# xcompact3d/x3d2

Hardware: AMD Instinct MI355X
Metric: DoF*steps/s (whole node), TGV 512^3 per GPU, full fractional step (higher is better)
Workload: dtype f64; 1 GPU; TGV 512x512x512 all-periodic, Re=1600, dt=1e-3, RK3 (3 substeps/step), compact6/classic schemes, rocFFT Poisson (configs[2]); per_gpu=512^3, driver=fused, parallelism=domain decomposition 1x1x1, decomposition=yslabs, decomposition_requested=auto, poisson_z_first=228

## Files before the change

### include/x3d2_hip.h

```cpp
#ifndef X3D2_HIP_H
#define X3D2_HIP_H

#include <stddef.h>

#ifdef X3D_SINGLE_PREC
typedef float x3d_real;
#else
typedef double x3d_real;
#endif

#ifdef __cplusplus
extern "C" {
#endif

enum { X3D_DIR_X = 1, X3D_DIR_Y = 2, X3D_DIR_Z = 3, X3D_DIR_C = 4 };
enum { X3D_BC_PERIODIC = 0, X3D_BC_NEUMANN = 1, X3D_BC_DIRICHLET = 2, X3D_BC_HALO = -1 };
enum { X3D_X_FACE = 1100, X3D_Y_FACE = 1010, X3D_Z_FACE = 110 };
#define X3D_N_HALO 4

typedef struct x3d_backend x3d_backend;
typedef struct x3d_tdsops x3d_tdsops;
typedef struct x3d_poisson x3d_poisson;

const char *x3d_last_error(void);
// ... 198 lines not shown
int x3d_poisson_postprocess_010(x3d_poisson *p);
int x3d_poisson_solve_010(x3d_poisson *p, x3d_real *f, x3d_real *temp);
int x3d_poisson_solve_010_rows(x3d_poisson *p, x3d_real *f);
int x3d_transpose_xy(x3d_backend *b_src, x3d_backend *b_dst, x3d_real *dst, const x3d_real *src, int nx, int ny, int nz);
int x3d_transpose_xyz_zxy(x3d_backend *b_src, x3d_backend *b_dst, x3d_real *dst, const x3d_real *src, int nx, int ny, int nz);
int x3d_transpose_zxy_xyz(x3d_backend *b_src, x3d_backend *b_dst, x3d_real *dst, const x3d_real *src, int nx, int ny, int nz);
int x3d_poisson_enforce_periodicity_z(x3d_poisson *p, x3d_real *f_out, const x3d_real *f_in);
int x3d_poisson_undo_periodicity_z(x3d_poisson *p, x3d_real *f_out, const x3d_real *f_in);
int x3d_poisson_postprocess_011(x3d_poisson *p);
int x3d_poisson_get_spectral(x3d_poisson *p, x3d_real *host_interleaved);
int x3d_poisson_set_spectral(x3d_poisson *p, const x3d_real *host_interleaved);

typedef struct x3d_sfft x3d_sfft;
int x3d_sfft_create(x3d_backend *b, x3d_sfft **out, const int nglob[3], int pz, int rz);
int x3d_sfft_destroy(x3d_sfft *p);
int x3d_sfft_sizes(const x3d_sfft *p, long out[4]);
int x3d_sfft_set_waves(x3d_sfft *p, const x3d_real *waves, const x3d_real *ax, const x3d_real *bx, const x3d_real *ay,
                       const x3d_real *by, const x3d_real *az, const x3d_real *bz);
int x3d_sfft_forward_local(x3d_sfft *p, const x3d_real *f_in, x3d_real *sendbuf);
int x3d_sfft_fft_z(x3d_sfft *p, x3d_real *recvbuf, int dir);
int x3d_sfft_postprocess_000(x3d_sfft *p, x3d_real *recvbuf);
int x3d_sfft_backward_local(x3d_sfft *p, const x3d_real *recvbuf, x3d_real *f_out);
int x3d_sfft_create_parts(x3d_backend *b, x3d_sfft **out, const int nglob[3], int pz, int rz, int parts);
int x3d_sfft_fft_z_part(x3d_sfft *p, x3d_real *recvbuf, int dir, int part);
int x3d_sfft_postprocess_000_part(x3d_sfft *p, x3d_real *recvbuf, int part);

typedef struct x3d_sfft010 x3d_sfft010;
int x3d_sfft010_create(x3d_backend *b, x3d_sfft010 **out, const int nglob_cell[3], int pz, int rz);
int x3d_sfft010_destroy(x3d_sfft010 *p);
int x3d_sfft010_sizes(const x3d_sfft010 *p, long out[6]);
int x3d_sfft010_create_parts(x3d_backend *b, x3d_sfft010 **out, const int nglob_cell[3], int pz, int rz, int parts);
int x3d_sfft010_fft_z_part(x3d_sfft010 *p, x3d_real *recvbuf, int dir, int part);
int x3d_sfft010_postprocess_010_part(x3d_sfft010 *p, x3d_real *recvbuf, int part);
int x3d_sfft010_set_waves(x3d_sfft010 *p, const x3d_real *waves, const x3d_real *ax, const x3d_real *bx, const x3d_real *ay,
                          const x3d_real *by, const x3d_real *az, const x3d_real *bz);
int x3d_sfft010_set_stretching(x3d_sfft010 *p, int sym, const x3d_real *a0, const x3d_real *a1);
int x3d_sfft010_periodicity_y(x3d_sfft010 *p, x3d_real *f_out, const x3d_real *f_in, int undo);
int x3d_sfft010_forward_local(x3d_sfft010 *p, const x3d_real *f_in, x3d_real *sendbuf);
int x3d_sfft010_fft_z(x3d_sfft010 *p, x3d_real *recvbuf, int dir);
int x3d_sfft010_postprocess_010(x3d_sfft010 *p, x3d_real *recvbuf);
int x3d_sfft010_backward_local(x3d_sfft010 *p, const x3d_real *sendbuf, x3d_real *f_out);

int x3d_poisson_zfirst_ok(x3d_poisson *p, int *ok);
int x3d_tds_pair_zfirst_ok(x3d_backend *b, const x3d_tdsops *ta, const x3d_tdsops *tb, int *ok);
int x3d_poisson_zfirst_middle(x3d_poisson *p);
int x3d_poisson_zfirst_forward(x3d_poisson *p, const x3d_real *f_in);
int x3d_poisson_zfirst_backward(x3d_poisson *p, x3d_real *f_out);
int x3d_poisson_solve_000_zfirst(x3d_poisson *p, x3d_real *f);
int x3d_tds_solve_xfft_ok(x3d_backend *b, const x3d_tdsops *t, int *ok);
int x3d_tds_solve_xfft(x3d_backend *b, x3d_real *du, const x3d_real *u, const x3d_tdsops *t);
int x3d_poisson_xfft_ok(x3d_poisson *p, int *ok);
int x3d_poisson_zfirst_middle_xpacked(x3d_poisson *p);
int x3d_c2c512_x_rows(x3d_backend *b, x3d_real *c, long nrows, long pitch, int mode);
int x3d_poisson_set_stretching_zfirst(x3d_poisson *p, int sym, const x3d_real *a0, const x3d_real *a1);
int x3d_poisson_create_proxy(x3d_backend *b, x3d_poisson **out, x3d_real *spectrum, int ny, long px, int (*middle)(void *user),
                             void *user);
int x3d_poisson_solve_010_rows_zfirst(x3d_poisson *p, x3d_real *f);
int x3d_tds_pair_zfirst(x3d_backend *b, x3d_poisson *poisson, int mode, x3d_real *out1, x3d_real *out2, const x3d_real *in1,
                        const x3d_real *in2, const x3d_tdsops *ta, const x3d_tdsops *tb, int *done);

typedef struct x3d_sfftz x3d_sfftz;
int x3d_sfftz_create(x3d_backend *b, x3d_sfftz **out, const int nglob_cell[3], int py, int ry, int parts);
int x3d_sfftz_destroy(x3d_sfftz *p);
int x3d_sfftz_sizes(const x3d_sfftz *p, long out[16]);
int x3d_sfftz_spectrum(const x3d_sfftz *p, x3d_real **c, int *ny, long *px);
int x3d_sfftz_set_waves(x3d_sfftz *p, const x3d_real *rw, const x3d_real *ax, const x3d_real *bx, const x3d_real *ay,
                        const x3d_real *by, const x3d_real *az, const x3d_real *bz);
int x3d_sfftz_tds_pair(x3d_sfftz *p, int mode, x3d_real *out1, x3d_real *out2, const x3d_real *in1, const x3d_real *in2,
                       const x3d_tdsops *ta, const x3d_tdsops *tb, int *done);
int x3d_sfftz_z(x3d_sfftz *p, x3d_real *f, int inverse);
int x3d_sfftz_z_field(x3d_sfftz *p, x3d_real *f, int inverse);
int x3d_sfftz_x_forward(x3d_sfftz *p, x3d_real *sendbuf, int part);
int x3d_sfftz_y_stage(x3d_sfftz *p, x3d_real *recvbuf, int part, int what);
int x3d_sfftz_x_backward(x3d_sfftz *p, const x3d_real *buf, int part);
int x3d_sfftz_tds_pair_rows(x3d_sfftz *p, int mode, x3d_real *out1, x3d_real *out2, const x3d_real *in1, const x3d_real *in2,
                            const x3d_tdsops *ta, const x3d_tdsops *tb, int y0, int nyr, int *done);
int x3d_sfftz_z_rows(x3d_sfftz *p, x3d_real *f, int inverse, int y0, int nyr);
int x3d_sfftz_x_forward_rows(x3d_sfftz *p, x3d_real *sendbuf, int part, int y0, int nyr);
int x3d_sfftz_x_backward_rows(x3d_sfftz *p, const x3d_real *buf, int part, int y0, int nyr);

typedef struct x3d_pfft x3d_pfft;
int x3d_pfft_create(x3d_backend *b, x3d_pfft **out, const int nglob_cell[3], int py, int pz, int ry, int rz);
int x3d_pfft_destroy(x3d_pfft *p);
int x3d_pfft_sizes(const x3d_pfft *p, long out[8]);
int x3d_pfft_set_waves(x3d_pfft *p, const x3d_real *waves_re, const x3d_real *ax, const x3d_real *bx,
                       const x3d_real *ay, const x3d_real *by, const x3d_real *az, const x3d_real *bz);
int x3d_pfft_fwd_x(x3d_pfft *p, const x3d_real *f_in);
int x3d_pfft_bwd_x(x3d_pfft *p, x3d_real *f_out);
int x3d_pfft_fft_y(x3d_pfft *p, int inverse);
int x3d_pfft_fft_z(x3d_pfft *p, int inverse);
int x3d_pfft_pack_xy(x3d_pfft *p, x3d_real *sendbuf);
int x3d_pfft_unpack_xy(x3d_pfft *p, const x3d_real *recvbuf);
int x3d_pfft_pack_yx(x3d_pfft *p, x3d_real *sendbuf);
int x3d_pfft_unpack_yx(x3d_pfft *p, const x3d_real *recvbuf);
int x3d_pfft_pack_yz(x3d_pfft *p, x3d_real *sendbuf);
int x3d_pfft_unpack_yz(x3d_pfft *p, const x3d_real *recvbuf);
int x3d_pfft_pack_zy(x3d_pfft *p, x3d_real *sendbuf);
int x3d_pfft_unpack_zy(x3d_pfft *p, const x3d_real *recvbuf);
int x3d_pfft_transpose_local(x3d_pfft *p, int which);
int x3d_pfft_own_chunk(x3d_pfft *p, const x3d_real *sendbuf, int rank);
int x3d_pfft_postprocess_000(x3d_pfft *p);
int x3d_pfft_create_parts(x3d_backend *b, x3d_pfft **out, const int nglob_cell[3], int py, int pz, int ry, int rz,
                          int parts);
int x3d_pfft_part_layout(const x3d_pfft *p, long out[6]);
int x3d_pfft_fwd_a_part(x3d_pfft *p, const x3d_real *f_in, x3d_real *send_xy, int m);
int x3d_pfft_fwd_b_part(x3d_pfft *p, const x3d_real *recv_xy, x3d_real *send_yz, int m);
// ... 128 lines not shown
```

### x3d2_amd/_lib.py

```python
import ctypes
import os
import subprocess

from .common import X3dError

HERE = os.path.dirname(os.path.abspath(__file__))
SINGLE = os.environ.get("X3D_SINGLE_PREC") == "1"
LIB_PATH = os.path.join(HERE, "libx3d2_hip_sp.so" if SINGLE else "libx3d2_hip.so")
CSRC = os.path.join(HERE, "csrc")

REAL = ctypes.c_float if SINGLE else ctypes.c_double
NP_REAL = "float32" if SINGLE else "float64"
c_double_p = ctypes.POINTER(REAL)
c_int_p = ctypes.POINTER(ctypes.c_int)
VP = ctypes.c_void_p
I, D, SZT = ctypes.c_int, REAL, ctypes.c_size_t


def torch_real():
    import torch
    return torch.float32 if SINGLE else torch.float64

PROTOTYPES = {
    "x3d_last_error": (ctypes.c_char_p, []),
# ... 108 lines not shown
    "x3d_get_field_data_pitched": (I, [VP, c_double_p, VP, I, I, c_int_p]),
    "x3d_poisson_create": (I, [VP, ctypes.POINTER(VP), c_int_p] + [c_double_p] * 7),
    "x3d_poisson_destroy": (I, [VP]),
    "x3d_poisson_fft_forward": (I, [VP, VP]),
    "x3d_poisson_postprocess_000": (I, [VP]),
    "x3d_poisson_fft_backward": (I, [VP, VP]),
    "x3d_poisson_solve_000": (I, [VP, VP]),
    "x3d_poisson_enforce_periodicity_y": (I, [VP, VP, VP]),
    "x3d_poisson_undo_periodicity_y": (I, [VP, VP, VP]),
    "x3d_poisson_set_stretching": (I, [VP, ctypes.c_int, c_double_p, c_double_p]),
    "x3d_sfftz_spectrum": (I, [VP, ctypes.POINTER(VP), c_int_p, ctypes.POINTER(ctypes.c_long)]),
    "x3d_poisson_create_proxy": (I, [VP, ctypes.POINTER(VP), VP, I, ctypes.c_long, VP, VP]),
    "x3d_poisson_set_stretching_zfirst": (I, [VP, ctypes.c_int, c_double_p, c_double_p]),
    "x3d_poisson_postprocess_010": (I, [VP]),
    "x3d_poisson_solve_010": (I, [VP, VP, VP]),
    "x3d_poisson_solve_010_rows": (I, [VP, VP]),
    "x3d_poisson_solve_010_rows_zfirst": (I, [VP, VP]),
    "x3d_poisson_get_spectral": (I, [VP, c_double_p]),
    "x3d_poisson_set_spectral": (I, [VP, c_double_p]),
    "x3d_sfft_create": (I, [VP, ctypes.POINTER(VP), c_int_p, I, I]),
    "x3d_sfft_create_parts": (I, [VP, ctypes.POINTER(VP), c_int_p, I, I, I]),
    "x3d_sfft_fft_z_part": (I, [VP, VP, I, I]),
    "x3d_sfft_postprocess_000_part": (I, [VP, VP, I]),
    "x3d_sfft_destroy": (I, [VP]),
    "x3d_sfft_sizes": (I, [VP, ctypes.POINTER(ctypes.c_long)]),
    "x3d_sfft_set_waves": (I, [VP] + [c_double_p] * 7),
    "x3d_sfft_forward_local": (I, [VP, VP, VP]),
    "x3d_sfft_fft_z": (I, [VP, VP, I]),
    "x3d_sfft_postprocess_000": (I, [VP, VP]),
    "x3d_sfft_backward_local": (I, [VP, VP, VP]),
    "x3d_sfft010_create": (I, [VP, ctypes.POINTER(VP), c_int_p, I, I]),
    "x3d_sfft010_create_parts": (I, [VP, ctypes.POINTER(VP), c_int_p, I, I, I]),
    "x3d_sfft010_fft_z_part": (I, [VP, VP, I, I]),
    "x3d_sfft010_postprocess_010_part": (I, [VP, VP, I]),
    "x3d_sfft010_destroy": (I, [VP]),
    "x3d_sfft010_sizes": (I, [VP, ctypes.POINTER(ctypes.c_long)]),
    "x3d_sfft010_set_waves": (I, [VP] + [c_double_p] * 7),
    "x3d_sfft010_set_stretching": (I, [VP, I, c_double_p, c_double_p]),
    "x3d_sfft010_periodicity_y": (I, [VP, VP, VP, I]),
    "x3d_sfft010_forward_local": (I, [VP, VP, VP]),
    "x3d_sfft010_fft_z": (I, [VP, VP, I]),
    "x3d_sfft010_postprocess_010": (I, [VP, VP]),
    "x3d_sfft010_backward_local": (I, [VP, VP, VP]),
    "x3d_poisson_zfirst_ok": (I, [VP, c_int_p]),
    "x3d_poisson_zfirst_middle": (I, [VP]),
    "x3d_poisson_zfirst_forward": (I, [VP, VP]),
    "x3d_poisson_zfirst_backward": (I, [VP, VP]),
    "x3d_poisson_solve_000_zfirst": (I, [VP, VP]),
    "x3d_tds_solve_xfft_ok": (I, [VP, VP, c_int_p]),
    "x3d_tds_solve_xfft": (I, [VP, VP, VP, VP]),
    "x3d_poisson_xfft_ok": (I, [VP, c_int_p]),
    "x3d_poisson_zfirst_middle_xpacked": (I, [VP]),
    "x3d_c2c512_x_rows": (I, [VP, VP, ctypes.c_long, ctypes.c_long, I]),
    "x3d_tds_pair_zfirst": (I, [VP, VP, I, VP, VP, VP, VP, VP, VP, c_int_p]),
    "x3d_sfftz_create": (I, [VP, ctypes.POINTER(VP), c_int_p, I, I, I]),
    "x3d_sfftz_destroy": (I, [VP]),
    "x3d_sfftz_sizes": (I, [VP, ctypes.POINTER(ctypes.c_long)]),
    "x3d_sfftz_set_waves": (I, [VP] + [c_double_p] * 7),
    "x3d_sfftz_tds_pair": (I, [VP, I, VP, VP, VP, VP, VP, VP, c_int_p]),
    "x3d_sfftz_z": (I, [VP, VP, I]),
    "x3d_sfftz_z_field": (I, [VP, VP, I]),
    "x3d_sfftz_x_forward": (I, [VP, VP, I]),
    "x3d_sfftz_y_stage": (I, [VP, VP, I, I]),
    "x3d_sfftz_x_backward": (I, [VP, VP, I]),
    "x3d_sfftz_tds_pair_rows": (I, [VP, I, VP, VP, VP, VP, VP, VP, I, I, c_int_p]),
    "x3d_sfftz_z_rows": (I, [VP, VP, I, I, I]),
    "x3d_sfftz_x_forward_rows": (I, [VP, VP, I, I, I]),
    "x3d_sfftz_x_backward_rows": (I, [VP, VP, I, I, I]),
    "x3d_pfft_create": (I, [VP, ctypes.POINTER(VP), c_int_p, I, I, I, I]),
    "x3d_pfft_destroy": (I, [VP]),
    "x3d_pfft_sizes": (I, [VP, ctypes.POINTER(ctypes.c_long)]),
    "x3d_pfft_set_waves": (I, [VP] + [c_double_p] * 7),
    "x3d_pfft_fwd_x": (I, [VP, VP]),
    "x3d_pfft_bwd_x": (I, [VP, VP]),
    "x3d_pfft_fft_y": (I, [VP, I]),
    "x3d_pfft_fft_z": (I, [VP, I]),
    "x3d_pfft_pack_xy": (I, [VP, VP]),
    "x3d_pfft_unpack_xy": (I, [VP, VP]),
    "x3d_pfft_pack_yx": (I, [VP, VP]),
    "x3d_pfft_unpack_yx": (I, [VP, VP]),
    "x3d_pfft_pack_yz": (I, [VP, VP]),
    "x3d_pfft_unpack_yz": (I, [VP, VP]),
    "x3d_pfft_pack_zy": (I, [VP, VP]),
    "x3d_pfft_unpack_zy": (I, [VP, VP]),
    "x3d_pfft_transpose_local": (I, [VP, I]),
    "x3d_pfft_own_chunk": (I, [VP, VP, I]),
    "x3d_pfft_postprocess_000": (I, [VP]),
    "x3d_pfft_create_parts": (I, [VP, ctypes.POINTER(VP), c_int_p, I, I, I, I, I]),
    "x3d_pfft_part_layout": (I, [VP, ctypes.POINTER(ctypes.c_long)]),
    "x3d_pfft_fwd_a_part": (I, [VP, VP, VP, I]),
    "x3d_pfft_fwd_b_part": (I, [VP, VP, VP, I]),
    "x3d_pfft_fwd_c_part": (I, [VP, VP, I]),
    "x3d_pfft_bwd_c_part": (I, [VP, VP, I]),
    "x3d_pfft_bwd_b_part": (I, [VP, VP, VP, I]),
    "x3d_pfft_bwd_a_part": (I, [VP, VP, VP, I]),
    "x3d_stats_update_uvw": (I, [VP, VP, VP, VP, ctypes.POINTER(VP), D]),
    "x3d_stats_update_scalar": (I, [VP, VP, VP, VP, D]),
    "x3d_stats_derive": (I, [VP, ctypes.POINTER(VP), ctypes.POINTER(VP)]),
    "x3d_stats_profile_sums": (I, [VP, VP, VP, VP, c_int_p, I, VP]),
    "x3d_stats_profile_accumulate": (I, [VP, VP, VP, ctypes.c_long, D, D]),
    "x3d_ibm_create": (I, [VP, c_double_p, c_int_p, ctypes.POINTER(VP)]),
    "x3d_ibm_destroy": (I, [VP]),
    "x3d_ibm_counts": (I, [VP, ctypes.POINTER(ctypes.c_long)]),
    "x3d_ibm_body": (I, [VP, VP, VP, VP, VP, c_int_p]),
    "x3d_ibm_set_weights": (I, [VP] + [ctypes.POINTER(ctypes.c_double)] * 3),
    "x3d_ibm_body_loads": (I, [VP, VP, VP, VP, VP, c_int_p, VP, I]),
# ... 96 lines not shown
```

### x3d2_amd/backend.py

```python
import ctypes

import numpy as np
import torch

from . import _lib
from .common import (CELL, DIR_C, DIR_X, DIR_Y, DIR_Z, N_HALO, NULL_LOC, VERT, X_FACE, Y_FACE, Z_FACE, X3dError,
                     get_rdr_from_dirs, move_data_loc)
from .field import Allocator
from .parallel import Comm
from .switches import Switches
from .tdsops import Tdsops

VP = ctypes.c_void_p


def _dp(a):
    if a.dtype != np.dtype(_lib.NP_REAL):
        a = np.ascontiguousarray(a, dtype=_lib.NP_REAL)
    return a.ctypes.data_as(_lib.c_double_p)


class HipBackend:
    n_halo = N_HALO

# ... 415 lines not shown
            else:
                for j in jobs:
                    self.tds_job_local(direction, j)
                if after_lead:
                    after_lead()
            if between:
                between()
            return
        if direction != DIR_X and all(self.tds_tile_ok(direction, j, True, yperm=yperm) for j in jobs):
            hs = [self.tds_halo_begin(direction, j, k) for k, j in enumerate(jobs)]
            hb = [self.tds_halo_main(direction, j, k, hs[k], yperm=yperm) for k, j in enumerate(jobs)]
            if after_lead:
                after_lead()
            if between:
                between()
            for k, j in enumerate(jobs):
                self.tds_halo_finish(direction, j, k, hb[k], yperm=yperm)
            return
        if yperm:
            raise X3dError("tds_jobs: interleaved rows need the halo form of the z pairs (tds_tile_ok)")
        for j in jobs:
            self.tds_job_local(direction, j)
        if after_lead:
            after_lead()
        if between:
            between()

    def halo_strip_rows(self, *ops):
        out = (ctypes.c_int * 2)()
        ws = we = 0
        for t in ops:
            _lib.check(self.lib.x3d_tdsops_halo_rows(t.handle, out))
            ws, we = max(ws, out[0]), max(we, out[1])
        return ws, we

    def transeq_dir(self, direction, du, dv, dw, u, v, w, nu, dirps, accumulate=False):
        if not self._decomposed(direction):
            _lib.check(self.lib.x3d_transeq_acc(self.h, direction, du.ptr, dv.ptr, dw.ptr, u.ptr, v.ptr, w.ptr,
                                                float(nu), dirps.der1st.handle, dirps.der1st_sym.handle,
                                                dirps.der2nd.handle, dirps.der2nd_sym.handle, int(accumulate)))
            return
        self._transeq_dist(direction, du, dv, dw, u, v, w, nu, dirps, accumulate=accumulate)

    def transeq_x_update(self, du, dv, dw, u, v, w, nu, dirps, grads, op_u, op_vw, scale):
        if self._decomposed(DIR_X):
            return False
        flag = ctypes.c_int(0)
        _lib.check(self.lib.x3d_transeq_x_update(self.h, du.ptr, dv.ptr, dw.ptr, u.ptr, v.ptr, w.ptr, float(nu),
                                                 dirps.der1st.handle, dirps.der1st_sym.handle, dirps.der2nd.handle,
                                                 dirps.der2nd_sym.handle, grads[0].ptr, grads[1].ptr, grads[2].ptr,
                                                 op_u.handle, op_vw.handle, float(scale), ctypes.byref(flag)))
        return bool(flag.value)

    def transeq_x_update_rot(self, du, dv, dw, u, v, w, nu, dirps, grads, op_u, op_vw, scale, omega, u_shift=None):
        if self._decomposed(DIR_X):
            return False
        flag = ctypes.c_int(0)
        _lib.check(self.lib.x3d_transeq_x_update_rot(self.h, du.ptr, dv.ptr, dw.ptr, u.ptr, v.ptr, w.ptr, float(nu),
                                                     dirps.der1st.handle, dirps.der1st_sym.handle, dirps.der2nd.handle,
                                                     dirps.der2nd_sym.handle, grads[0].ptr, grads[1].ptr, grads[2].ptr,
                                                     op_u.handle, op_vw.handle, float(scale), float(omega), u_shift,
                                                     ctypes.byref(flag)))
        return bool(flag.value)

    def transeq_x_rot(self, du, dv, dw, u, v, w, nu, dirps, omega, u_shift=None):
        if self._decomposed(DIR_X):
            return False
        flag = ctypes.c_int(0)
        _lib.check(self.lib.x3d_transeq_x_rot(self.h, du.ptr, dv.ptr, dw.ptr, u.ptr, v.ptr, w.ptr, float(nu),
                                              dirps.der1st.handle, dirps.der1st_sym.handle, dirps.der2nd.handle,
                                              dirps.der2nd_sym.handle, float(omega), u_shift, ctypes.byref(flag)))
        return bool(flag.value)

    def transeq_dir_defer(self, direction, pend, u, v, w, nu, dirps):
        if self._decomposed(direction):
            return False
        flag = ctypes.c_int(0)
        _lib.check(self.lib.x3d_transeq_defer(self.h, direction, pend[0].ptr, pend[1].ptr, pend[2].ptr, u.ptr, v.ptr,
                                              w.ptr, float(nu), dirps.der1st.handle, dirps.der1st_sym.handle,
                                              dirps.der2nd.handle, dirps.der2nd_sym.handle, ctypes.byref(flag)))
        return bool(flag.value)

    def transeq_stage_ok(self, direction, dirps):
        if self._decomposed(direction):
            return False
        return bool(self.lib.x3d_transeq_stage_ok(self.h, direction, dirps.der1st.handle, dirps.der1st_sym.handle,
                                                  dirps.der2nd.handle, dirps.der2nd_sym.handle))

    def transeq_lincomb(self, direction, kind, u_ptr, conv_ptr, nu, dirps, y, base, coeffs, xs, ipend, store):
        n = len(xs)
        c = (_lib.REAL * n)(*[float(v) for v in coeffs])
        p = (VP * n)(*[x.ptr for x in xs])
        _lib.check(self.lib.x3d_transeq_lincomb(self.h, direction, int(kind), u_ptr, conv_ptr, float(nu),
                                                dirps.der1st.handle, dirps.der1st_sym.handle, dirps.der2nd.handle,
                                                dirps.der2nd_sym.handle, y.ptr, base.ptr, n, c, p, int(ipend),
                                                int(bool(store))))
        self.rk_fused_passes = getattr(self, "rk_fused_passes", 0) + n + 1
        self.rk_fused_launches = getattr(self, "rk_fused_launches", 0) + 1

    def transeq_lincomb3(self, direction, rhs, vel, nu, dirps, specs):
        y = (VP * 3)(*[sp[0].ptr for sp in specs])
        base = (VP * 3)(*[sp[1].ptr for sp in specs])
        nterm = _lib.ints(*[len(sp[3]) for sp in specs])
        c = (_lib.REAL * 15)()
        x = (VP * 15)()
        ipend, store = [], []
# ... 65 lines not shown
            if mode == 0:
                self.tds_apply(out1, in2, t_b, direction, accumulate=True)
            else:
                self.tds_apply(out2, in1, t_b, direction)
            return
        _lib.check(self.lib.x3d_tds_solve_pair(self.h, direction, int(mode), out1.ptr,
                                               out2.ptr if out2 is not None else None, in1.ptr,
                                               in2.ptr if in2 is not None else None, t_a.handle, t_b.handle))

    def tds_pair_yperm(self, mode, out1, out2, in1, in2, t_a, t_b, ny):
        if self._decomposed(DIR_Z) or self.sw.no_yperm:
            return False
        flag = ctypes.c_int(0)
        _lib.check(self.lib.x3d_tds_solve_pair_yperm(self.h, int(mode), out1.ptr,
                                                     out2.ptr if out2 is not None else None, in1.ptr,
                                                     in2.ptr if in2 is not None else None, t_a.handle, t_b.handle,
                                                     int(ny), ctypes.byref(flag)))
        return bool(flag.value)

    def tds_pair_zfirst(self, mode, out1, out2, in1, in2, t_a, t_b):
        if self._decomposed(DIR_Z) or self.poisson_fft is None or not hasattr(self.poisson_fft, "zfirst_ok"):
            return False
        if hasattr(self.poisson_fft, "zfirst_pair"):
            return self.poisson_fft.zfirst_pair(mode, out1, out2, in1, in2, t_a, t_b)
        flag = ctypes.c_int(0)
        ptr = lambda f: f.ptr if f is not None else None
        _lib.check(self.lib.x3d_tds_pair_zfirst(self.h, self.poisson_fft.h, int(mode), ptr(out1), ptr(out2), ptr(in1),
                                                ptr(in2), t_a.handle, t_b.handle, ctypes.byref(flag)))
        return bool(flag.value)

    def zfirst_pairs_ok(self, t_a, t_b):
        flag = ctypes.c_int(0)
        _lib.check(self.lib.x3d_tds_pair_zfirst_ok(self.h, t_a.handle, t_b.handle, ctypes.byref(flag)))
        return bool(flag.value)

    def tds_apply_mean(self, du, u, tdsops, direction, mean_target):
        if u.data_loc == NULL_LOC:
            raise X3dError("You must set the data_loc before calling volume integral.")
        out = VP()
        ncell = float(np.prod(self.mesh.get_global_dims(CELL)))
        _lib.check(self.lib.x3d_tds_solve_mean(self.h, du.ptr, u.ptr, tdsops.handle, direction, self._dims(u.data_loc), ncell,
                                               float(mean_target), ctypes.byref(out)))
        return out

    def tds_apply_xfft_ok(self, tdsops):
        if self._decomposed(DIR_X):
            return False
        flag = ctypes.c_int(0)
        _lib.check(self.lib.x3d_tds_solve_xfft_ok(self.h, tdsops.handle, ctypes.byref(flag)))
        return bool(flag.value)

    def tds_apply_xfft(self, du, u, tdsops):
        _lib.check(self.lib.x3d_tds_solve_xfft(self.h, du.ptr, u.ptr, tdsops.handle))

    def tds_apply(self, du, u, tdsops, direction, accumulate=False, scale=1.0):
        if not self._decomposed(direction):
            _lib.check(self.lib.x3d_tds_solve_acc(self.h, du.ptr, u.ptr, tdsops.handle, direction,
                                                  int(accumulate), float(scale)))
            return
        self._tds_dist(du, u, tdsops, direction, accumulate=accumulate, scale=scale)

    def tds_solve(self, du, u, tdsops):
        if u.dir != du.dir:
            raise X3dError("DIR mismatch between fields in tds_solve.")
        if u.data_loc != NULL_LOC:
            du.set_data_loc(move_data_loc(u.data_loc, u.dir, tdsops.move))
        direction = u.dir
        if direction == DIR_C:
            raise X3dError("tds_solve needs a directional field")
        if tdsops.pentadiag:
            self.tds_penta_solve(du, u, tdsops, direction)
            return
        if not self._decomposed(direction):
            _lib.check(self.lib.x3d_tds_solve(self.h, du.ptr, u.ptr, tdsops.handle, direction))
            return
        self._tds_dist(du, u, tdsops, direction)

    def tds_penta_solve(self, du, u, tdsops, direction, u_s=None, u_e=None):
        if self._decomposed(direction):
            raise X3dError("compact10_penta is a rank-local solve: the direction must not be decomposed")
        _lib.check(self.lib.x3d_tds_penta_solve(self.h, du.ptr, u.ptr, tdsops.handle, direction,
                                                u_s.data_ptr() if u_s is not None else None,
                                                u_e.data_ptr() if u_e is not None else None))

    def _tds_dist(self, du, u, tdsops, direction, accumulate=False, scale=1.0):
        if not accumulate and direction != DIR_X:
            job = (2, du, None, u, None, tdsops, None)
            if self.tds_tile_ok(direction, job, True):
                h = self.tds_halo_begin(direction, job, 0)
                hb = self.tds_halo_main(direction, job, 0, h)
                self.tds_halo_finish(direction, job, 0, hb)
                return
        d = direction - 1
        prev, nxt = int(self.mesh.pprev[d]), int(self.mesh.pnext[d])
        ss, se, rs, re = self._buffers(direction, N_HALO, "u0")
        _lib.check(self.lib.x3d_pack_halos(self.h, ss.data_ptr(), se.data_ptr(), u.ptr, tdsops.n_tds,
                                           direction))
        self.comm.sendrecv([(ss, se, rs, re)], prev, nxt)
        bs, be, brs, bre = self._buffers(direction, 1, "b1")
        _lib.check(self.lib.x3d_tds_dist_fwd(self.h, du.ptr, bs.data_ptr(), be.data_ptr(), u.ptr,
                                             rs.data_ptr(), re.data_ptr(), tdsops.handle, direction))
        self.comm.sendrecv([(bs, be, brs, bre)], prev, nxt)
        _lib.check(self.lib.x3d_tds_dist_bwd_acc(self.h, du.ptr, bs.data_ptr(), brs.data_ptr(), bre.data_ptr(),
                                                 tdsops.handle, direction, int(bool(accumulate)), float(scale)))

    def reorder(self, u_, u, direction):
# ... 423 lines not shown
```

### x3d2_amd/csrc/common.h

```cpp
#pragma once
#include <hip/hip_runtime.h>

#include <cstdarg>
#include <cstdio>
#include <cstring>
#include <vector>

#include "../../include/x3d2_hip.h"

typedef x3d_real real_t;
#ifdef X3D_SINGLE_PREC
typedef float2 real2_t;
#define make_real2 make_float2
#else
typedef double2 real2_t;
#define make_real2 make_double2
#endif
#ifdef X3D_SINGLE_PREC
#define X3D_FFT_R2C HIPFFT_R2C
#define X3D_FFT_C2R HIPFFT_C2R
#define X3D_FFT_C2C HIPFFT_C2C
#define x3d_fftExecR2C hipfftExecR2C
#define x3d_fftExecC2R hipfftExecC2R
#define x3d_fftExecC2C hipfftExecC2C
// ... 32 lines not shown
            x3d_set_error(__VA_ARGS__);                                                        \
            return 2;                                                                          \
        }                                                                                      \
    } while (0)

__device__ __forceinline__ double fma_r(double a, double b, double c) { return __builtin_fma(a, b, c); }
__device__ __forceinline__ float fma_r(float a, float b, float c) { return __builtin_fmaf(a, b, c); }

__device__ __forceinline__ void wave_lds_fence()
{
    __builtin_amdgcn_fence(__ATOMIC_RELEASE, "wavefront");
    __builtin_amdgcn_wave_barrier();
    __builtin_amdgcn_fence(__ATOMIC_ACQUIRE, "wavefront");
}

typedef real_t x3d_d2v __attribute__((ext_vector_type(2)));
__device__ __forceinline__ real2_t ldg_stream(const real2_t *p)
{
    const x3d_d2v v = __builtin_nontemporal_load(reinterpret_cast<const x3d_d2v *>(p));
    return make_real2(v.x, v.y);
}
__device__ __forceinline__ void stg_stream(real2_t *p, real2_t v)
{
    const x3d_d2v w = {v.x, v.y};
    __builtin_nontemporal_store(w, reinterpret_cast<x3d_d2v *>(p));
}

static __device__ __attribute__((used)) float g_vmcnt_sink[32 * 1024];
template <int N>
__device__ __forceinline__ void vmcnt_pad_stores()
{
#pragma unroll
    for (int k = 0; k < N; k++) __builtin_nontemporal_store(0.0f, &g_vmcnt_sink[k * 1024 + (threadIdx.x & 1023)]);
}

__host__ __device__ static inline unsigned long long x3d_mix64(unsigned long long z)
{
    z += 0x9E3779B97F4A7C15ull;
    z = (z ^ (z >> 30)) * 0xBF58476D1CE4E5B9ull;
    z = (z ^ (z >> 27)) * 0x94D049BB133111EBull;
    return z ^ (z >> 31);
}

struct PencilGeom {
    int np;
    int dim0;
    long s0, s1, rs;
};

#define X3D_SW_UNSET (-0x7fffffffL - 1)
struct x3d_switches {
    long no_via_x, no_xscan, no_ygen, no_ytile, no_q5, no_direct, sfft010_split_xy;
    long no_circ, no_halo_circ, no_uniform, xscan_p1, no_ztile, no_tds_pair, no_npw2, no_tile3, xdir_generic, no_xcirc;
    long no_tds_lincomb, no_zfirst010, no_zfirst, no_xwide, no_xwide_upd, no_xfft_div;
    long no_spectral_pad, no_fft512, no_rwt, no_r2c512, no_y010, y010_no_db, no_onchip2, no_slab_fused_z;
    long lazy_dump, lazy_report, lazy_keep_zero_terms;
    long pad_x;
    long slab_z_split;
    long lazy_rules;
    long y010_form;
    long via_x;
    long ytile;
    long ygen;
    long x_fast;
    long x_tq3;
    long x_circ;
};
void x3d_switches_from_env(x3d_switches *sw);

struct x3d_backend {
    x3d_switches sw;
    int device;
    hipStream_t stream;
    int nx, ny, nz;
    int ring[4];
    int nxp, nyp, nzp;
    size_t nblock;
    real_t *send_s, *send_e;
    real_t *scratch[3];
    real_t *red_buf;
    real_t *red_host;
    int red_cap;
    long n_upd;
    long n_tq3;
    long n_halo;
    void *epi_dev;
    hipEvent_t ev0, ev1;
    void *ipc_maps;
    struct x3d_prof *prof;
    unsigned prof_mask;
    int pair_yperm;
    void *lds_optin;
    struct x3d_lazy *lazy;
    int comm_reserve;
    double *stats_part;
    long stats_cap;
    real_t *bc_params;
    double *bc_part;
    long n_sync;
    void *snap;
};
void x3d_snapshot_destroy_c(x3d_backend *b);
int x3d_snapshot_wait_for_copy_c(x3d_backend *b, const void *dev);
int x3d_reduce_abs_partials_c(x3d_backend *b, const real_t *f, const int dims[3], int *nparts);
#define X3D_BC_PARTS 1024
struct TileEpi {
    real_t *y;
// ... 175 lines not shown
```

### x3d2_amd/csrc/fft512_core.h

```cpp
#pragma once
#include "common.h"

#define FP 584

__device__ __forceinline__ real2_t cmul(real2_t a, real2_t b)
{
    return make_real2(a.x * b.x - a.y * b.y, a.x * b.y + a.y * b.x);
}
__device__ __forceinline__ real2_t cadd(real2_t a, real2_t b) { return make_real2(a.x + b.x, a.y + b.y); }
__device__ __forceinline__ real2_t csub(real2_t a, real2_t b) { return make_real2(a.x - b.x, a.y - b.y); }

template <int S>
__device__ __forceinline__ void fft8(real2_t (&a)[8])
{
    const real_t h = 0.70710678118654752440;
    real2_t b[8];
#pragma unroll
    for (int k = 0; k < 4; k++) {
        b[k] = cadd(a[k], a[k + 4]);
        b[k + 4] = csub(a[k], a[k + 4]);
    }
    {
        real2_t t = b[5];
        b[5] = make_real2(h * (t.x - S * t.y), h * (t.y + S * t.x));
// ... 66 lines not shown
{
    const real2_t b0 = cadd(a[0], a[2]), b1 = csub(a[0], a[2]), b2 = cadd(a[1], a[3]), d = csub(a[1], a[3]);
    const real2_t b3 = make_real2(-S * d.y, S * d.x);
    a[0] = cadd(b0, b2);
    a[2] = csub(b0, b2);
    a[1] = cadd(b1, b3);
    a[3] = csub(b1, b3);
}

template <int S>
__device__ __forceinline__ void fft256_wave(real2_t (&a)[4], real2_t *__restrict__ pen, const real2_t *__restrict__ tw,
                                            int l)
{
    wave_lds_fence();
    fft4<S>(a);
#pragma unroll
    for (int f = 1; f < 4; f++) a[f] = cmul(a[f], twiddle<S>(tw, 2 * l * f));
#pragma unroll
    for (int f = 0; f < 4; f++) pen[f * 68 + l] = a[f];
    wave_lds_fence();
    {
        const int f1 = l >> 4, l0 = l & 15;
#pragma unroll
        for (int j = 0; j < 4; j++) a[j] = pen[f1 * 68 + l0 + 16 * j];
        fft4<S>(a);
#pragma unroll
        for (int f = 1; f < 4; f++) a[f] = cmul(a[f], twiddle<S>(tw, 8 * l0 * f));
        wave_lds_fence();
#pragma unroll
        for (int f = 0; f < 4; f++) pen[(f1 * 4 + f) * 17 + l0] = a[f];
    }
    wave_lds_fence();
    {
        const int r = l >> 2, m0 = l & 3;
#pragma unroll
        for (int m = 0; m < 4; m++) a[m] = pen[r * 17 + m0 + 4 * m];
        fft4<S>(a);
#pragma unroll
        for (int f = 1; f < 4; f++) a[f] = cmul(a[f], twiddle<S>(tw, 32 * m0 * f));
        wave_lds_fence();
#pragma unroll
        for (int f = 0; f < 4; f++) pen[(r * 4 + f) * 4 + m0 + (r >> 2) * 4] = a[f];
    }
    wave_lds_fence();
    {
        const int f1 = l & 3, f2 = (l >> 2) & 3, f3 = l >> 4;
        const int row = ((f1 * 4 + f2) * 4 + f3) * 4 + f1 * 4;
#pragma unroll
        for (int m = 0; m < 4; m++) a[m] = pen[row + m];
        fft4<S>(a);
    }
    wave_lds_fence();
}
```

### x3d2_amd/csrc/switches.hip

```cpp
#include <cstdlib>

#include "common.h"

enum SwKind {
    SW_FLAG,
    SW_INT,
    SW_MASK,
    SW_FORM,
};
struct SwEntry {
    const char *name;
    SwKind kind;
    long unset;
    long x3d_switches::*field;
};
#define F(name, field) {name, SW_FLAG, 0, &x3d_switches::field}
static const SwEntry g_table[] = {
    F("X3D_NO_XSCAN", no_xscan),
    F("X3D_XDIR_GENERIC", xdir_generic),
    F("X3D_XSCAN_P1", xscan_p1),
    F("X3D_NO_TILE3", no_tile3),
    F("X3D_NO_XCIRC", no_xcirc),
    F("X3D_NO_CIRC", no_circ),
    F("X3D_NO_HALO_CIRC", no_halo_circ),
    F("X3D_NO_UNIFORM", no_uniform),
    F("X3D_NO_TDS_LINCOMB", no_tds_lincomb),
    F("X3D_NO_XWIDE", no_xwide),
    F("X3D_NO_XWIDE_UPD", no_xwide_upd),
    F("X3D_NO_VIA_X", no_via_x),
    F("X3D_NO_YTILE", no_ytile),
    F("X3D_NO_ZTILE", no_ztile),
    F("X3D_NO_YGEN", no_ygen),
    F("X3D_NO_Q5", no_q5),
    F("X3D_NO_DIRECT", no_direct),
    F("X3D_NO_TDS_PAIR", no_tds_pair),
    F("X3D_NO_NPW2", no_npw2),
    F("X3D_NO_ONCHIP2", no_onchip2),
    F("X3D_NO_SPECTRAL_PAD", no_spectral_pad),
    F("X3D_NO_FFT512", no_fft512),
    F("X3D_NO_RWT", no_rwt),
    F("X3D_NO_R2C512", no_r2c512),
    F("X3D_NO_ZFIRST", no_zfirst),
    F("X3D_NO_XFFT_DIV", no_xfft_div),
    F("X3D_NO_ZFIRST010", no_zfirst010),
    F("X3D_NO_Y010", no_y010),
    F("X3D_Y010_NO_DB", y010_no_db),
    F("X3D_SFFT010_SPLIT_XY", sfft010_split_xy),
    F("X3D_NO_SLAB_FUSED_Z", no_slab_fused_z),
    F("X3D_LAZY_DUMP", lazy_dump),
    F("X3D_LAZY_REPORT", lazy_report),
    F("X3D_LAZY_KEEP_ZERO_TERMS", lazy_keep_zero_terms),
    {"X3D_LAZY_RULES", SW_MASK, 0xffffffffL, &x3d_switches::lazy_rules},
    {"X3D_PAD_X", SW_INT, X3D_SW_UNSET, &x3d_switches::pad_x},
    {"X3D_SLAB_Z_SPLIT", SW_INT, -1, &x3d_switches::slab_z_split},
    {"X3D_Y010_FORM", SW_FORM, 1, &x3d_switches::y010_form},
};
#undef F

static long resolve(const SwEntry &s)
{
    const char *e = getenv(s.name);
    switch (s.kind) {
    case SW_FLAG: return e && e[0] == '1';
    case SW_INT: return e ? atoi(e) : s.unset;
    case SW_MASK: return e ? (long)(unsigned)strtoul(e, nullptr, 0) : s.unset;
    default: return !e || !e[0] ? s.unset : (e[0] == 's' && e[1] == 't' ? 1 : 0);
    }
}

void x3d_switches_from_env(x3d_switches *sw)
{
    for (const SwEntry &s : g_table) sw->*s.field = resolve(s);
    sw->via_x = !(sw->no_via_x || sw->no_xscan);
    sw->ytile = sw->via_x && !sw->no_ytile;
    sw->ygen = sw->ytile && !sw->no_ygen;
    sw->x_fast = !(sw->no_xscan || sw->xdir_generic);
    sw->x_tq3 = sw->x_fast && !(sw->no_tile3 || sw->xscan_p1);
    sw->x_circ = !(sw->no_circ || sw->no_xcirc);
}

extern "C" int x3d_backend_switch(const x3d_backend *b, const char *name, long *value)
{
    X3D_REQUIRE(name && value, "x3d_backend_switch: null argument");
    for (const SwEntry &s : g_table)
        if (!strcmp(s.name, name)) {
            *value = b ? b->sw.*s.field : resolve(s);
            return 0;
        }
    x3d_set_error("x3d_backend_switch: %s is not a switch of the library", name);
    return 2;
}
```

### x3d2_amd/csrc/tds.hip

```cpp
#include "common.h"
#include "zfft_tile.h"

extern "C" int x3d_tdsops_create(x3d_backend *b, x3d_tdsops **out, int n_tds, int n_rhs, int move,
                                 int periodic, const real_t *coeffs, const real_t *coeffs_s,
                                 const real_t *coeffs_e, const real_t *dist_fw, const real_t *dist_bw,
                                 const real_t *dist_sa, const real_t *dist_sc, const real_t *dist_af,
                                 const real_t *stretch, const real_t *stretch_correct)
{
    X3D_RANGE(__func__);
    X3D_REQUIRE(b && out && coeffs && coeffs_s && coeffs_e && dist_fw && dist_bw && dist_sa && dist_sc &&
                    dist_af && stretch && stretch_correct,
                "x3d_tdsops_create: null argument");
    X3D_REQUIRE(n_rhs == n_tds || n_rhs == n_tds + 1, "x3d_tdsops_create: n_rhs must be n_tds or n_tds+1");
    X3D_REQUIRE(n_tds >= 8, "x3d_tdsops_create: n_tds=%d too small (the 4+4 boundary rows need n>=8)", n_tds);
    const int n = n_tds, nr = n_rhs, L = nr + 2;
    std::vector<real_t> h((size_t)10 * L + 81, 0.0);
    real_t *F = &h[0], *A = &h[L], *W = &h[2 * L], *Bw = &h[3 * L], *Sa = &h[4 * L], *Sc = &h[5 * L],
           *St = &h[6 * L], *Stc = &h[7 * L], *PF = &h[8 * L], *QB = &h[9 * L], *Cs = &h[10 * L];
    for (int j = 1; j <= nr; j++) {
        const bool real_row = j <= n;
        if (j <= 2) {
            F[j] = dist_af[j - 1];
            A[j] = 0.0;
        } else {
// ... 722 lines not shown
                             const real_t *__restrict__ u, int n, PencilGeom g)
{
    const int p = blockIdx.x * blockDim.x + threadIdx.x;
    if (p >= g.np) return;
    const long base = pencil_base(g, p);
#pragma unroll
    for (int r = 0; r < X3D_NH; r++) {
        send_s[(long)r * g.np + p] = u[base + (long)r * g.rs];
        send_e[(long)r * g.np + p] = u[base + (long)(n - X3D_NH + r) * g.rs];
    }
}

struct PackFields { const real_t *f[3]; };
__global__ void k_pack_halos_multi(real_t *__restrict__ send, PackFields pf, int nf, int n, PencilGeom g, int hp, long hnp)
{
    const int p = blockIdx.x * blockDim.x + threadIdx.x;
    if (p >= g.np) return;
    const long base = pencil_base(g, p);
    const long hq = (long)(p / g.dim0) * hp + p % g.dim0;
    const int k = blockIdx.y;
    const real_t *__restrict__ u = pf.f[k];
#pragma unroll
    for (int r = 0; r < X3D_NH; r++) {
        send[((long)k * X3D_NH + r) * hnp + hq] = u[base + (long)r * g.rs];
        send[((long)(nf + k) * X3D_NH + r) * hnp + hq] = u[base + (long)(n - X3D_NH + r) * g.rs];
    }
}

void x3d_halo_layout(const x3d_backend *b, int dir, int *hp, long *hnp)
{
    if (dir == X3D_DIR_Z) { *hp = b->nxp; *hnp = (long)b->nxp * b->nyp; }
    else { *hp = b->nx; *hnp = (long)x3d_geom(b, dir).np; }
}
extern "C" long x3d_halo_row_size(const x3d_backend *b, int dir)
{
    X3D_RANGE(__func__);
    if (!b || !x3d_dir_ok(dir)) return 0;
    int hp;
    long hnp;
    x3d_halo_layout(b, dir, &hp, &hnp);
    return hnp;
}

int x3d_onchip2_tds(x3d_backend *b, real_t *du, const real_t *u, const x3d_tdsops *t, int dir, int acc, real_t scale,
                    bool *done);
int x3d_transeq_via_x(x3d_backend *b, int dir, real_t *const r[3], const real_t *const f[3], real_t nu,
                      const x3d_tdsops *der1st, const x3d_tdsops *der1st_sym, const x3d_tdsops *der2nd,
                      const x3d_tdsops *der2nd_sym, int acc, bool *done);
int x3d_ytile_transeq(x3d_backend *b, int dir, real_t *rhs, const real_t *u, const real_t *conv, real_t nu,
                      const x3d_tdsops *t1, const x3d_tdsops *t2, const x3d_tdsops *t3, int acc, bool *done);
int x3d_xscan_transeq3(x3d_backend *b, real_t *const r[3], const real_t *const f[3], real_t nu,
                       const x3d_tdsops *der1st, const x3d_tdsops *der1st_sym, const x3d_tdsops *der2nd,
                       const x3d_tdsops *der2nd_sym, int acc, const real_t *const *upd_g, const x3d_tdsops *op_s,
                       const x3d_tdsops *op_i, real_t scale, real_t omega, const real_t *ushift, bool *done);
int x3d_xwide_transeq3_upd(x3d_backend *b, real_t *const r[3], real_t *const f[3], real_t nu, const x3d_tdsops *der1st,
                           const x3d_tdsops *der1st_sym, const x3d_tdsops *der2nd, const x3d_tdsops *der2nd_sym,
                           const real_t *const g[3], const x3d_tdsops *op_s, const x3d_tdsops *op_i, real_t scale,
                           real_t omega, const real_t *ushift, bool *done);
int x3d_xwide_transeq3(x3d_backend *b, real_t *const r[3], const real_t *const f[3], real_t nu, const x3d_tdsops *der1st,
                       const x3d_tdsops *der1st_sym, const x3d_tdsops *der2nd, const x3d_tdsops *der2nd_sym, int acc,
                       real_t omega, const real_t *ushift, bool *done);
int x3d_ygen_pair(x3d_backend *b, int dir, int mode, real_t *out1, real_t *out2, const real_t *in1, const real_t *in2,
                  const x3d_tdsops *ta, const x3d_tdsops *tb, bool *done);
int x3d_ygen_transeq3(x3d_backend *b, int dir, real_t *const r[3], const real_t *const f[3], real_t nu,
                      const x3d_tdsops *der1st, const x3d_tdsops *der1st_sym, const x3d_tdsops *der2nd,
                      const x3d_tdsops *der2nd_sym, int acc, bool *done);
int x3d_xdir_tds(x3d_backend *b, real_t *du, const real_t *u, const x3d_tdsops *t, int acc, real_t scale);
int x3d_xdir_transeq(x3d_backend *b, real_t *rhs, const real_t *u, const real_t *conv, real_t nu,
                     const x3d_tdsops *t1, const x3d_tdsops *t2, const x3d_tdsops *t3, int acc);
int x3d_generic_tds_local(x3d_backend *b, real_t *du, const real_t *u, const x3d_tdsops *t, int dir, int acc,
                          real_t scale);
int x3d_generic_transeq_local(x3d_backend *b, int dir, real_t *rhs, const real_t *u, const real_t *conv,
                              real_t nu, const x3d_tdsops *t1, const x3d_tdsops *t2, const x3d_tdsops *t3,
                              int acc);

static inline dim3 grid_for(const PencilGeom &g) { return dim3((g.np + 63) / 64); }

static int check_len(const x3d_backend *b, const x3d_tdsops *t, int dir, const char *who)
{
    const int ext = dir == X3D_DIR_X ? b->nx : (dir == X3D_DIR_Y ? b->ny : b->nz);
    X3D_REQUIRE(t->n_rhs <= ext, "%s: operator needs %d rows but the block has %d along dir %d", who, t->n_rhs,
                ext, dir);
    return 0;
}

extern "C" int x3d_pack_halos(x3d_backend *b, real_t *send_s, real_t *send_e, const real_t *u, int n, int dir)
{
    X3D_RANGE(__func__);
    X3D_REQUIRE(b && send_s && send_e && u, "x3d_pack_halos: null argument");
    X3D_LAZY_IN(b, u);
    X3D_LAZY_EAGER(b);
    X3D_REQUIRE(x3d_dir_ok(dir), "x3d_pack_halos: bad dir %d", dir);
    PencilGeom g = x3d_geom(b, dir);
    ProfScope ps(b, X3D_K_PACK, dir);
    hipLaunchKernelGGL(k_pack_halos, dim3((g.np + 255) / 256), dim3(256), 0, b->stream, send_s, send_e, u, n, g);
    X3D_HIP(hipGetLastError());
    return 0;
}

extern "C" int x3d_tds_dist_fwd(x3d_backend *b, real_t *du, real_t *du_send_s, real_t *du_send_e,
                                const real_t *u, const real_t *u_recv_s, const real_t *u_recv_e,
                                const x3d_tdsops *t, int dir)
{
    X3D_RANGE(__func__);
    X3D_REQUIRE(b && du && du_send_s && du_send_e && u && u_recv_s && u_recv_e && t,
                "x3d_tds_dist_fwd: null argument");
    X3D_REQUIRE(x3d_dir_ok(dir), "x3d_tds_dist_fwd: bad dir %d", dir);
// ... 30 lines not shown
    X3D_HIP(hipGetLastError());
    return 0;
}

extern "C" int x3d_tds_dist_bwd(x3d_backend *b, real_t *du, const real_t *du_send_s, const real_t *du_recv_s,
                                const real_t *du_recv_e, const x3d_tdsops *t, int dir)
{
    X3D_RANGE(__func__);
    return x3d_tds_dist_bwd_acc(b, du, du_send_s, du_recv_s, du_recv_e, t, dir, 0, 1.0);
}

extern "C" int x3d_tds_solve_acc(x3d_backend *b, real_t *du, const real_t *u, const x3d_tdsops *t, int dir,
                                 int accumulate, real_t scale)
{
    X3D_RANGE(__func__);
    if (b) X3D_LAZY_SYNC(b);
    X3D_LAZY_EAGER(b);
    X3D_REQUIRE(b && du && u && t, "x3d_tds_solve: null argument");
    X3D_REQUIRE(x3d_dir_ok(dir), "x3d_tds_solve: bad dir %d", dir);
    X3D_REQUIRE(du != u, "x3d_tds_solve: du and u must be distinct blocks");
    if (int rc = check_len(b, t, dir, "tds_solve")) return rc;
    if (dir == X3D_DIR_X) return x3d_xdir_tds(b, du, u, t, accumulate, scale);
    if (!b->sw.no_onchip2) {
        bool done = false;
        if (int rc = x3d_onchip2_tds(b, du, u, t, dir, accumulate, scale, &done)) return rc;
        if (done) return 0;
    }
    if (!accumulate) {
        bool done = false;
        if (int rc = x3d_ygen_pair(b, dir, 2, du, nullptr, u, nullptr, t, t, &done)) return rc;
        if (done) return 0;
    }
    return x3d_generic_tds_local(b, du, u, t, dir, accumulate, scale);
}

bool x3d_xscan_tds_xfft_ok(const x3d_backend *b, const x3d_tdsops *t);
int x3d_xscan_tds_xfft(x3d_backend *b, real_t *du, const real_t *u, const x3d_tdsops *t);
extern "C" int x3d_tds_solve_xfft_ok(x3d_backend *b, const x3d_tdsops *t, int *ok)
{
    X3D_RANGE(__func__);
    X3D_REQUIRE(b && t && ok, "x3d_tds_solve_xfft_ok: null argument");
    *ok = x3d_xscan_tds_xfft_ok(b, t) ? 1 : 0;
    return 0;
}
extern "C" int x3d_tds_solve_xfft(x3d_backend *b, real_t *du, const real_t *u, const x3d_tdsops *t)
{
    X3D_RANGE(__func__);
    if (b) X3D_LAZY_SYNC(b);
    X3D_LAZY_EAGER(b);
    X3D_REQUIRE(b && du && u && t, "x3d_tds_solve_xfft: null argument");
    X3D_REQUIRE(du != u, "x3d_tds_solve_xfft: du and u must be distinct blocks");
    if (int rc = check_len(b, t, X3D_DIR_X, "tds_solve_xfft")) return rc;
    return x3d_xscan_tds_xfft(b, du, u, t);
}

int x3d_ytile_tds_pair(x3d_backend *b, int dir, int mode, real_t *out1, real_t *out2, const real_t *in1, const real_t *in2,
                       const x3d_tdsops *ta, const x3d_tdsops *tb, const TileHalo *halo, int other0, int nother,
                       bool *done);
int x3d_tds_halo_fix(x3d_backend *b, int dir, int mode, real_t *out1, real_t *out2, const real_t *brecv,
                     const x3d_tdsops *ta, const x3d_tdsops *tb);
int x3d_transeq_halo_fix_launch(x3d_backend *b, int dir, real_t *const r[3], const real_t *conv, real_t nu,
                                const real_t *brecv, const x3d_tdsops *der1st, const x3d_tdsops *der2nd);
int x3d_ytile_transeq3(x3d_backend *b, int dir, real_t *const r[3], const real_t *const f[3], real_t nu,
                       const x3d_tdsops *der1st, const x3d_tdsops *der1st_sym, const x3d_tdsops *der2nd,
                       const x3d_tdsops *der2nd_sym, int acc, const TileHalo *halo, int other0, int nother,
                       bool *done);

extern "C" int x3d_tds_solve_pair(x3d_backend *b, int dir, int mode, real_t *out1, real_t *out2, const real_t *in1,
                                  const real_t *in2, const x3d_tdsops *ta, const x3d_tdsops *tb)
{
    X3D_RANGE(__func__);
    if (b) X3D_LAZY_SYNC(b);
    X3D_LAZY_EAGER(b);
    X3D_REQUIRE(b && out1 && in1 && ta && tb && (mode == 0 ? in2 != nullptr : out2 != nullptr),
                "x3d_tds_solve_pair: null argument");
    X3D_REQUIRE(mode == 0 || mode == 1, "x3d_tds_solve_pair: mode must be 0 or 1");
    X3D_REQUIRE(x3d_dir_ok(dir), "x3d_tds_solve_pair: bad dir %d", dir);
    X3D_REQUIRE(out1 != in1 && out1 != in2 && out2 != in1 && (mode == 0 || out1 != out2),
                "x3d_tds_solve_pair: outputs alias inputs");
    if (int rc = check_len(b, ta, dir, "tds_solve_pair")) return rc;
    if (int rc = check_len(b, tb, dir, "tds_solve_pair")) return rc;
    if (dir != X3D_DIR_X) {
        bool done = false;
        if (int rc = x3d_ytile_tds_pair(b, dir, mode, out1, out2, in1, in2, ta, tb, nullptr, 0, -1, &done)) return rc;
        if (done) return 0;
        if (int rc = x3d_ygen_pair(b, dir, mode, out1, out2, in1, in2, ta, tb, &done)) return rc;
        if (done) return 0;
    }
    if (int rc = x3d_tds_solve_acc(b, out1, in1, ta, dir, 0, 1.0)) return rc;
    return mode == 0 ? x3d_tds_solve_acc(b, out1, in2, tb, dir, 1, 1.0) : x3d_tds_solve_acc(b, out2, in1, tb, dir, 0, 1.0);
}

extern "C" int x3d_tds_solve_pair_yperm(x3d_backend *b, int mode, real_t *out1, real_t *out2, const real_t *in1,
                                        const real_t *in2, const x3d_tdsops *ta, const x3d_tdsops *tb, int ny, int *done)
{
    X3D_RANGE(__func__);
    if (b) X3D_LAZY_SYNC(b);
    X3D_LAZY_EAGER(b);
    X3D_REQUIRE(b && out1 && in1 && ta && tb && done && (mode == 0 ? in2 != nullptr : out2 != nullptr),
                "x3d_tds_solve_pair_yperm: null argument");
    X3D_REQUIRE(mode == 0 || mode == 1, "x3d_tds_solve_pair_yperm: mode must be 0 or 1");
    X3D_REQUIRE(out1 != in1 && out1 != in2 && out2 != in1 && (mode == 0 || out1 != out2),
                "x3d_tds_solve_pair_yperm: outputs alias inputs");
    X3D_REQUIRE(ny > 0 && ny <= b->ny, "x3d_tds_solve_pair_yperm: ny = %d outside the block (%d rows)", ny, b->ny);
    *done = 0;
    if (int rc = check_len(b, ta, X3D_DIR_Z, "tds_solve_pair_yperm")) return rc;
// ... 314 lines not shown
        if (done) return 0;
    }
    if (dir != X3D_DIR_X) {
        bool done = false;
        if (int rc = x3d_transeq_via_x(b, dir, r, f, nu, der1st, der1st_sym, der2nd, der2nd_sym, a, &done)) return rc;
        if (done) return 0;
    }
    if (dir != X3D_DIR_X) {
        bool done = false;
        if (int rc = x3d_ygen_transeq3(b, dir, r, f, nu, der1st, der1st_sym, der2nd, der2nd_sym, a, &done)) return rc;
        if (done) return 0;
    }
    if (int rc = transeq_component_local(b, dir, r[0], f[0], f[0], nu, der1st, der1st_sym, der2nd, a)) return rc;
    if (int rc = transeq_component_local(b, dir, r[1], f[1], f[0], nu, der1st_sym, der1st, der2nd_sym, a)) return rc;
    if (int rc = transeq_component_local(b, dir, r[2], f[2], f[0], nu, der1st_sym, der1st, der2nd_sym, a)) return rc;
    return 0;
}

extern "C" int x3d_transeq_x_update(x3d_backend *b, real_t *du, real_t *dv, real_t *dw, real_t *u, real_t *v, real_t *w,
                                    real_t nu, const x3d_tdsops *der1st, const x3d_tdsops *der1st_sym,
                                    const x3d_tdsops *der2nd, const x3d_tdsops *der2nd_sym, const real_t *gu,
                                    const real_t *gv, const real_t *gw, const x3d_tdsops *op_u,
                                    const x3d_tdsops *op_vw, real_t scale, int *done)
{
    X3D_RANGE(__func__);
    if (b) X3D_LAZY_SYNC(b);
    X3D_LAZY_EAGER(b);
    X3D_REQUIRE(b && du && dv && dw && u && v && w && der1st && der1st_sym && der2nd && der2nd_sym && gu && gv && gw &&
                    op_u && op_vw && done,
                "x3d_transeq_x_update: null argument");
    *done = 0;
    if (int rc = transeq_check(b, X3D_DIR_X, der1st, der1st_sym, der2nd)) return rc;
    if (int rc = check_len(b, op_u, X3D_DIR_X, "transeq_x_update")) return rc;
    if (int rc = check_len(b, op_vw, X3D_DIR_X, "transeq_x_update")) return rc;
    real_t *r[3] = {du, dv, dw};
    const real_t *f[3] = {u, v, w}, *g[3] = {gu, gv, gw};
    for (int c = 0; c < 3; c++)
        for (int k = 0; k < 3; k++)
            X3D_REQUIRE(r[c] != f[k] && r[c] != g[k] && f[c] != g[k], "x3d_transeq_x_update: arguments alias");
    bool ok = false;
    if (int rc = x3d_xscan_transeq3(b, r, f, nu, der1st, der1st_sym, der2nd, der2nd_sym, 0, g, op_u, op_vw, scale, 0.0,
                                    nullptr, &ok))
        return rc;
    if (!ok) {
        real_t *fw[3] = {u, v, w};
        if (int rc = x3d_xwide_transeq3_upd(b, r, fw, nu, der1st, der1st_sym, der2nd, der2nd_sym, g, op_u, op_vw, scale, 0.0,
                                            nullptr, &ok))
            return rc;
    }
    *done = ok ? 1 : 0;
    return 0;
}

extern "C" int x3d_transeq_x_update_rot(x3d_backend *b, real_t *du, real_t *dv, real_t *dw, real_t *u, real_t *v, real_t *w,
                                        real_t nu, const x3d_tdsops *der1st, const x3d_tdsops *der1st_sym,
                                        const x3d_tdsops *der2nd, const x3d_tdsops *der2nd_sym, const real_t *gu,
                                        const real_t *gv, const real_t *gw, const x3d_tdsops *op_u,
                                        const x3d_tdsops *op_vw, real_t scale, real_t omega, const real_t *u_shift, int *done)
{
    X3D_RANGE(__func__);
    if (omega == 0.0 && !u_shift)
        return x3d_transeq_x_update(b, du, dv, dw, u, v, w, nu, der1st, der1st_sym, der2nd, der2nd_sym, gu, gv, gw, op_u, op_vw,
                                    scale, done);
    if (b) X3D_LAZY_SYNC(b);
    X3D_LAZY_EAGER(b);
    X3D_REQUIRE(b && du && dv && dw && u && v && w && der1st && der1st_sym && der2nd && der2nd_sym && gu && gv && gw &&
                    op_u && op_vw && done,
                "x3d_transeq_x_update_rot: null argument");
    *done = 0;
    if (int rc = transeq_check(b, X3D_DIR_X, der1st, der1st_sym, der2nd)) return rc;
    if (int rc = transeq_check(b, X3D_DIR_X, der1st_sym, der1st, der2nd_sym)) return rc;
    if (int rc = check_len(b, op_u, X3D_DIR_X, "transeq_x_update_rot")) return rc;
    if (int rc = check_len(b, op_vw, X3D_DIR_X, "transeq_x_update_rot")) return rc;
    real_t *r[3] = {du, dv, dw}, *f[3] = {u, v, w};
    const real_t *g[3] = {gu, gv, gw};
    for (int c = 0; c < 3; c++)
        for (int k = 0; k < 3; k++)
            X3D_REQUIRE(r[c] != f[k] && r[c] != g[k] && f[c] != g[k], "x3d_transeq_x_update_rot: arguments alias");
    bool ok = false;
    if (int rc = x3d_xwide_transeq3_upd(b, r, f, nu, der1st, der1st_sym, der2nd, der2nd_sym, g, op_u, op_vw, scale, omega,
                                        u_shift, &ok))
        return rc;
    *done = ok ? 1 : 0;
    return 0;
}

extern "C" int x3d_transeq_x_rot(x3d_backend *b, real_t *du, real_t *dv, real_t *dw, real_t *u, const real_t *v,
                                 const real_t *w, real_t nu, const x3d_tdsops *der1st, const x3d_tdsops *der1st_sym,
                                 const x3d_tdsops *der2nd, const x3d_tdsops *der2nd_sym, real_t omega,
                                 const real_t *u_shift, int *done)
{
    X3D_RANGE(__func__);
    if (b) X3D_LAZY_SYNC(b);
    X3D_LAZY_EAGER(b);
    X3D_REQUIRE(b && du && dv && dw && u && v && w && der1st && der1st_sym && der2nd && der2nd_sym && done,
                "x3d_transeq_x_rot: null argument");
    *done = 0;
    if (int rc = transeq_check(b, X3D_DIR_X, der1st, der1st_sym, der2nd)) return rc;
    if (int rc = transeq_check(b, X3D_DIR_X, der1st_sym, der1st, der2nd_sym)) return rc;
    real_t *r[3] = {du, dv, dw};
    const real_t *f[3] = {u, v, w};
    for (int c = 0; c < 3; c++)
        X3D_REQUIRE(r[c] != f[0] && r[c] != f[1] && r[c] != f[2], "x3d_transeq_x_rot: outputs alias inputs");
    if (omega == 0.0 && !u_shift) return 0;
    bool ok = false;
    if (int rc = x3d_xscan_transeq3(b, r, f, nu, der1st, der1st_sym, der2nd, der2nd_sym, 0, nullptr, nullptr, nullptr, 0.0,
// ... 216 lines not shown
```

### x3d2_amd/csrc/xscan.hip

```cpp
#include "common.h"


int npmax_of(const x3d_backend *b);

#include "xscan_core.h"
#include "zfft_tile.h"


template <bool ACC>
__device__ __forceinline__ void store_rows_q8(real_t *__restrict__ orow, int lane, const real_t (&r)[8],
                                              real_t scale)
{
    const int j = lane & 3;
    real_t a0 = r[0], a1 = r[1], b0 = r[2], b1 = r[3], c0 = r[4], c1 = r[5], d0 = r[6], d1 = r[7];
    rotl_pairs(a0, a1, b0, b1, c0, c1, d0, d1, j);
    b0 = dpp_quad(b0, 1); b1 = dpp_quad(b1, 1);
    c0 = dpp_quad(c0, 2); c1 = dpp_quad(c1, 2);
    d0 = dpp_quad(d0, 3); d1 = dpp_quad(d1, 3);
    rotl_pairs(a0, a1, b0, b1, c0, c1, d0, d1, j);
    real2_t *__restrict__ o2 = reinterpret_cast<real2_t *>(orow + (lane & ~3) * 8) + j;
    real2_t v0, v1, v2, v3;
    if (ACC) {
        v0 = o2[0]; v1 = o2[4]; v2 = o2[8]; v3 = o2[12];
        v0.x += scale * a0; v0.y += scale * a1;
// ... 125 lines not shown
            }
        }
    }
}

__global__ void __launch_bounds__(512, 4) k_xscan_tds_xfft(real_t *__restrict__ du, const real_t *__restrict__ u, int np,
                                                           long pitch, CircOp co, const real2_t *__restrict__ twg)
{
    constexpr int Q = 8;
    extern __shared__ real2_t xf[];
    real2_t *__restrict__ tws = xf + 8 * FP256;
    if (threadIdx.x < 256) tws[threadIdx.x] = twg[threadIdx.x];
    __syncthreads();
    const int lane = threadIdx.x & 63;
    const int wave = __builtin_amdgcn_readfirstlane(threadIdx.x >> 6);
    real2_t *__restrict__ pen = xf + wave * FP256;
    const int nwaves = gridDim.x * (blockDim.x >> 6);
    const int p0 = blockIdx.x * (blockDim.x >> 6) + wave;
    const int wsw = (lane >> 2) & 3, rsw = (lane >> 4) & 3;
    real_t nb[Q];
    if (p0 < np) load_body<Q>(nb, u + (long)p0 * pitch, lane);
    for (int p = p0; p < np; p += nwaves) {
        real_t w[Q + 8], r[Q];
        window_from_body<Q>(w, nb, lane);
        if (p + nwaves < np) load_body<Q>(nb, u + (long)(p + nwaves) * pitch, lane);
        circ_solve<Q, true>(w, r, co, lane);
        wave_lds_fence();
#pragma unroll
        for (int q = 0; q < 4; q++) pen[4 * lane + (q ^ wsw)] = make_real2(r[2 * q], r[2 * q + 1]);
        wave_lds_fence();
        real2_t a[4], c[4];
#pragma unroll
        for (int k = 0; k < 4; k++) a[k] = pen[64 * k + ((lane & ~3) | ((lane & 3) ^ rsw))];
        fft256_wave<-1>(a, pen, tws, lane);
#pragma unroll
        for (int f = 0; f < 4; f++) pen[lane + 64 * f] = a[f];
        wave_lds_fence();
#pragma unroll
        for (int f = 0; f < 4; f++) c[f] = pen[(256 - lane - 64 * f) & 255];
        real2_t *__restrict__ o2 = reinterpret_cast<real2_t *>(du + (long)p * pitch);
#pragma unroll
        for (int f = 0; f < 4; f++) {
            const int k = lane + 64 * f;
            const real2_t wk = twiddle<-1>(tws, k);
            const real_t er = 0.5 * (a[f].x + c[f].x), ei = 0.5 * (a[f].y - c[f].y);
            const real_t dr = 0.5 * (a[f].y + c[f].y), di = 0.5 * (c[f].x - a[f].x);
            real2_t F = make_real2(er + (wk.x * dr - wk.y * di), ei + (wk.x * di + wk.y * dr));
            if (f == 0 && lane == 0) F = make_real2(a[0].x + a[0].y, a[0].x - a[0].y);
            o2[k] = F;
        }
    }
}

template <int Q, bool NARROW, bool CIRC = false>
__global__ void __launch_bounds__(512) k_xscan_tds_lin(real_t *__restrict__ du, LinRows lr, XOp t, int np, long pitch,
                                                       CircOp co)
{
    extern __shared__ real_t lt[];
    if constexpr (!CIRC) {
        for (int i = threadIdx.x; i < LT_N(Q) * 64; i += blockDim.x) lt[i] = t.TL[i];
        __syncthreads();
    }
    int lane = threadIdx.x & 63;
    const int wave = __builtin_amdgcn_readfirstlane(threadIdx.x >> 6);
    const int nwaves = gridDim.x * (blockDim.x >> 6);
    const int first = lane * Q + 1;
    for (int p = blockIdx.x * (blockDim.x >> 6) + wave; p < np; p += nwaves) {
        const long ro = (long)p * pitch;
        asm volatile("" : "+v"(lane));
        real_t b[Q];
        load_body<Q>(b, lr.base + ro, lane);
#pragma unroll
        for (int k = 0; k < 5; k++)
            if (k < lr.n) {
                real_t xk[Q];
                load_body<Q>(xk, lr.x[k] + ro, lane);
#pragma unroll
                for (int q = 0; q < Q; q++) b[q] = lr.c[k] * xk[q] + b[q];
            }
        if (lr.wall) {
            const int j = p % lr.ny;
            if (j == 0 || j == lr.ny - 1) load_body<Q>(b, lr.wall + ro, lane);
        }
        if constexpr (Q == 8) store_rows_q8<false>(lr.y + ro, lane, b, 1.0);
        else store_rows_q4<false>(lr.y + ro, lane, b, 1.0);
        real_t w[Q + 8], X[Q], du1, xn;
        window_from_body<Q>(w, b, lane);
        real_t r[Q];
        if constexpr (CIRC) {
            circ_solve<Q, NARROW>(w, r, co, lane);
        } else {
        scan_solve<Q, true, NARROW>(w, X, du1, xn, lt, t, lane, first);
        const real_t du_s = t.rs_s * (du1 - t.sa1 * xn), du_e = t.rs_e * (xn - t.scn * du1);
#pragma unroll
        for (int q = 0; q < Q; q++) {
            const real_t st = LTR(lt, LT_ST(q));
            r[q] = (X[q] - LTR(lt, LT_SA(q)) * du_s - LTR(lt, LT_SC(q)) * du_e) * st;
            if (q == 0) r[q] = (lane == 0) ? du_s * st : r[q];
            if (q == Q - 1) r[q] = (lane == 63) ? du_e * st : r[q];
        }
        }
        if constexpr (Q == 8) store_rows_q8<false>(du + ro, lane, r, 1.0);
        else store_rows_q4<false>(du + ro, lane, r, 1.0);
    }
}

// ... 164 lines not shown
                load_body<Q>(nua, u + (long)pn * pitch, lane);
                load_body<Q>(nub, u + (long)(pn + 1) * pitch, lane);
                if (!SAME) {
                    load_body<Q>(nca, cv + (long)pn * pitch, lane);
                    load_body<Q>(ncb, cv + (long)(pn + 1) * pitch, lane);
                }
            }
#pragma unroll
            for (int m = 0; m < Q + 8; m++) wp[m] = SAME ? wu[m] * wu[m] : wu[m] * wp[m];
        }
        auto solve_subs = [&](const V2 (&w)[Q + 8], V2 (&T)[Q], const real_t *__restrict__ l, const XOp &t) {
            V2 a, b;
            scan_solve<Q, true, NARROW, V2>(w, T, a, b, l, t, lane, first);
            const V2 s_ = t.rs_s * (a - t.sa1 * b), e_ = t.rs_e * (b - t.scn * a);
#pragma unroll
            for (int q = 0; q < Q; q++) {
                const real_t st = LTR(l, LT_ST(q));
                V2 x = st * (T[q] - LTR(l, LT_SA(q)) * s_ - LTR(l, LT_SC(q)) * e_);
                if (q == 0) x = (lane == 0) ? s_ * st : x;
                if (q == Q - 1) x = (lane == 63) ? e_ * st : x;
                T[q] = x;
            }
        };
        V2 r[Q], T[Q];
        solve_subs(wp, T, l2, t2);
#pragma unroll
        for (int q = 0; q < Q; q++) r[q] = T[q];
        asm volatile("" : "+v"(lane) : "v"(r[0].a));
        solve_subs(wu, T, l1, t1);
#pragma unroll
        for (int q = 0; q < Q; q++) r[q] = -0.5 * (vq[q] * T[q] + r[q]) + nu * (T[q] * LTR(l3, LT_STC(q)));
        asm volatile("" : "+v"(lane) : "v"(r[0].a));
        solve_subs(wu, T, l3, t3);
        real_t ra[Q], rb[Q];
#pragma unroll
        for (int q = 0; q < Q; q++) {
            const V2 v = r[q] + nu * T[q];
            ra[q] = v.a;
            rb[q] = v.b;
        }
        real_t *__restrict__ oa = rhs + (long)p * pitch, *__restrict__ ob = oa + pitch;
        if constexpr (Q == 8) { store_rows_q8<ACC>(oa, lane, ra, 1.0); store_rows_q8<ACC>(ob, lane, rb, 1.0); }
        else { store_rows_q4<ACC>(oa, lane, ra, 1.0); store_rows_q4<ACC>(ob, lane, rb, 1.0); }
    }
}

struct XUpd {
    const real_t *g[3];
    real_t scale;
    real_t omega;
    const real_t *ushift;
};

template <int Q, bool ACC, bool NARROW, bool UPD, bool CHN = false, bool CIRC = false>
__global__ void __launch_bounds__(512)
    k_xscan_transeq2x3(real_t *__restrict__ rhs0, real_t *__restrict__ rhs1, real_t *__restrict__ rhs2, real_t *u0,
                       real_t *u1, real_t *u2, XOp tD1, XOp tD2, int np, long pitch, real_t nu, XUpd upd, XOp tS,
                       XOp tI, Circ4 cc)
{
    extern __shared__ real_t lt[];
    constexpr int LNF = LT_N(Q) * 64, LNC = LT_NC(Q) * 64, L1N = UPD ? LNC : LNF;
    static_assert(!CIRC || NARROW, "CIRC: 5-tap stencils");
    if constexpr (!CIRC) {
        for (int i = threadIdx.x; i < L1N; i += blockDim.x) lt[i] = tD1.TL[i];
        for (int i = threadIdx.x; i < LNF; i += blockDim.x) lt[L1N + i] = tD2.TL[i];
        if (UPD) {
            for (int i = threadIdx.x; i < LNC; i += blockDim.x) {
                lt[L1N + LNF + i] = tS.TL[i];
                lt[L1N + LNF + LNC + i] = tI.TL[i];
            }
        }
        __syncthreads();
    }
    int lane = threadIdx.x & 63;
    const int wave = __builtin_amdgcn_readfirstlane(threadIdx.x >> 6);
    const int nwaves = gridDim.x * (blockDim.x >> 6);
    const int first = lane * Q + 1;
    const real_t *__restrict__ l1 = lt, *__restrict__ l3 = lt + L1N;
    real_t na[Q], nb[Q];
    const int pstart = 2 * (blockIdx.x * (blockDim.x >> 6) + wave);
    if (pstart < np) {
        load_body<Q>(na, u0 + (long)pstart * pitch, lane);
        load_body<Q>(nb, u0 + (long)(pstart + 1) * pitch, lane);
    }
    for (int p = pstart; p < np; p += 2 * nwaves) {
        V2 cb[Q];
#pragma unroll 1
        for (int c = 0; c < 3; c++) {
            asm volatile("" : "+v"(lane));
            V2 wu[Q + 8], wp[Q + 8];
            {
                V2 b2[Q];
#pragma unroll
                for (int q = 0; q < Q; q++) b2[q] = V2{na[q], nb[q]};
                const int pn = p + 2 * nwaves;
                {
                    const real_t *nsrc = c == 0 ? u1 + (long)p * pitch : (c == 1 ? u2 + (long)p * pitch
                                                                                 : u0 + (long)(pn < np ? pn : p) * pitch);
                    if (c < 2 || pn < np) {
                        load_body<Q>(na, nsrc, lane);
                        load_body<Q>(nb, nsrc + pitch, lane);
                    }
                }
                if constexpr (UPD) {
                    const real_t *gsrc = (c == 0 ? upd.g[0] : (c == 1 ? upd.g[1] : upd.g[2])) + (long)p * pitch;
                    real_t ga[Q], gb[Q];
                    load_body<Q>(ga, gsrc, lane);
                    load_body<Q>(gb, gsrc + pitch, lane);
                    V2 g2[Q], wg[Q + 8], X[Q], du1, xn;
#pragma unroll
                    for (int q = 0; q < Q; q++) g2[q] = V2{ga[q], gb[q]};
                    window_from_body<Q, V2>(wg, g2, lane);
                    if constexpr (CIRC) {
                        if (c == 0) circ_solve<Q, NARROW, V2>(wg, X, cc.o[2], lane);
                        else circ_solve<Q, NARROW, V2>(wg, X, cc.o[3], lane);
#pragma unroll
                        for (int q = 0; q < Q; q++) b2[q] = b2[q] + upd.scale * X[q];
                    } else {
                    const real_t *__restrict__ lg = lt + L1N + LNF + (c == 0 ? 0 : LNC);
                    const XOp &tg = c == 0 ? tS : tI;
                    scan_solve<Q, true, NARROW, V2>(wg, X, du1, xn, lg, tg, lane, first);
                    const V2 du_s = tg.rs_s * (du1 - tg.sa1 * xn), du_e = tg.rs_e * (xn - tg.scn * du1);
#pragma unroll
                    for (int q = 0; q < Q; q++) {
                        const real_t st = LTR(lg, LT_ST(q));
                        V2 r = (X[q] - LTR(lg, LT_SA(q)) * du_s - LTR(lg, LT_SC(q)) * du_e) * st;
                        if (q == 0) r = (lane == 0) ? du_s * st : r;
                        if (q == Q - 1) r = (lane == 63) ? du_e * st : r;
                        b2[q] = b2[q] + upd.scale * r;
                    }
                    }
                    real_t ua[Q], ub[Q];
#pragma unroll
                    for (int q = 0; q < Q; q++) { ua[q] = b2[q].a; ub[q] = b2[q].b; }
                    real_t *uw = (c == 0 ? u0 : (c == 1 ? u1 : u2)) + (long)p * pitch;
                    if constexpr (Q == 8) { store_rows_q8<false>(uw, lane, ua, 1.0); store_rows_q8<false>(uw + pitch, lane, ub, 1.0); }
                    else { store_rows_q4<false>(uw, lane, ua, 1.0); store_rows_q4<false>(uw + pitch, lane, ub, 1.0); }
                    asm volatile("" : "+v"(lane) : "v"(b2[0].a));
                }
                if (CHN && c == 0 && upd.ushift) {
                    const real_t ush = *upd.ushift;
                    real_t ua[Q], ub[Q];
#pragma unroll
                    for (int q = 0; q < Q; q++) {
                        b2[q].a += ush;
                        b2[q].b += ush;
                        ua[q] = b2[q].a;
                        ub[q] = b2[q].b;
                    }
                    real_t *uw = u0 + (long)p * pitch;
                    if constexpr (Q == 8) { store_rows_q8<false>(uw, lane, ua, 1.0); store_rows_q8<false>(uw + pitch, lane, ub, 1.0); }
                    else { store_rows_q4<false>(uw, lane, ua, 1.0); store_rows_q4<false>(uw + pitch, lane, ub, 1.0); }
                }
                if (c == 0) {
#pragma unroll
                    for (int q = 0; q < Q; q++) cb[q] = b2[q];
                }
                window_from_body<Q, V2>(wu, b2, lane);
                window_from_body<Q, V2>(wp, cb, lane);
#pragma unroll
                for (int m = 0; m < Q + 8; m++) wp[m] = wu[m] * wp[m];
            }
            auto solve_subs = [&](const V2 (&w)[Q + 8], V2 (&T)[Q], const real_t *__restrict__ l, const XOp &t) {
                if constexpr (CIRC) {
// ... 800 lines not shown
static bool xscan_ok_gen(const x3d_tdsops *t) { return xscan_ok(t) || (t->tab.TL != nullptr && t->tab.Q == 6); }

int x3d_xscan_tds(x3d_backend *b, real_t *du, const real_t *u, const x3d_tdsops *t, int acc, real_t scale, bool *done)
{
    *done = false;
    if (!xscan_ok_gen(t)) return 0;
    const int Q = t->tab.Q, np = b->ny * b->nz;
    const bool fast = t->tab.bulk_only && t->n_tds == 64 * Q && t->tab.n_rhs == t->n_tds && Q != 6;
    const bool narrow = stencil_narrow(t);
    const bool circ = fast && narrow && t->uniform && t->circ_ok && !b->sw.no_circ;
    const size_t lds = circ ? 0 : sizeof(real_t) * (LT_N(Q) * 64 + CS_N(Q));
    int blocks = (np + 7) / 8;
    const int cap = circ ? 1024 : 768;
    blocks = blocks > cap ? cap : blocks;
    ProfScope ps(b, X3D_K_TDS_FWD, X3D_DIR_X);
#define LAUNCH(Q_, A_, F_, SC_)                                                                                \
    hipLaunchKernelGGL((k_xscan_tds<Q_, A_, F_>), dim3(blocks), dim3(512), lds, b->stream, du, u, xop_of(t), np, \
                       (long)b->nxp, t->n_tds, SC_, t->circ)
#define PICK(Q_)                                                                                               \
    do {                                                                                                       \
        if (circ) { if (acc) LAUNCH(Q_, true, 3, scale); else LAUNCH(Q_, false, 3, 1.0); }                     \
        else if (fast && narrow) { if (acc) LAUNCH(Q_, true, 2, scale); else LAUNCH(Q_, false, 2, 1.0); }      \
        else if (fast) { if (acc) LAUNCH(Q_, true, 1, scale); else LAUNCH(Q_, false, 1, 1.0); }                \
        else { if (acc) LAUNCH(Q_, true, 0, scale); else LAUNCH(Q_, false, 0, 1.0); }                          \
    } while (0)
    if (Q == 8) PICK(8);
    else if (Q == 6) { if (acc) LAUNCH(6, true, 0, scale); else LAUNCH(6, false, 0, 1.0); }
    else PICK(4);
#undef PICK
#undef LAUNCH
    X3D_HIP(hipGetLastError());
    *done = true;
    return 0;
}

int x3d_fft512_init();
const real2_t *x3d_fft512_twiddles();
bool x3d_xscan_tds_xfft_ok(const x3d_backend *b, const x3d_tdsops *t)
{
    return sizeof(real_t) == 8 && b->sw.x_fast && !b->sw.no_xfft_div && b->nx == 512 && b->nxp % 2 == 0 && xscan_ok(t) && t->tab.Q == 8 &&
           t->tab.bulk_only && t->n_tds == 512 && t->tab.n_rhs == 512 && stencil_narrow(t) && t->uniform && t->circ_ok &&
           !b->sw.no_circ;
}
int x3d_xscan_tds_xfft(x3d_backend *b, real_t *du, const real_t *u, const x3d_tdsops *t)
{
    X3D_REQUIRE(x3d_xscan_tds_xfft_ok(b, t), "x3d_tds_solve_xfft: not on offer for this operator (x3d_tds_solve_xfft_ok)");
    if (int rc = x3d_fft512_init()) return rc;
    const int np = b->ny * b->nz;
    const size_t lds = sizeof(real2_t) * (8 * FP256 + 256);
    int blocks = (np + 7) / 8;
    blocks = blocks > 1024 ? 1024 : blocks;
    ProfScope ps(b, X3D_K_TDS_FWD, X3D_DIR_X);
    hipLaunchKernelGGL(k_xscan_tds_xfft, dim3(blocks), dim3(512), lds, b->stream, du, u, np, (long)b->nxp, t->circ,
                       x3d_fft512_twiddles());
    X3D_HIP(hipGetLastError());
    return 0;
}

template <int Q, bool SAME, bool ACC, int FAST>
static int launch_transeq(x3d_backend *b, real_t *rhs, const real_t *u, const real_t *conv, real_t nu,
                          const x3d_tdsops *t1, const x3d_tdsops *t2, const x3d_tdsops *t3, int np, int blocks,
                          size_t lds, long pitch)
{
    X3D_LDS_OPTIN(b, (k_xscan_transeq<Q, SAME, ACC, FAST>));
    hipLaunchKernelGGL((k_xscan_transeq<Q, SAME, ACC, FAST>), dim3(blocks), dim3(FAST ? 1024 : 512), lds, b->stream, rhs, u, conv, xop_of(t1),
                       xop_of(t2), xop_of(t3), np, pitch, nu);
    X3D_HIP(hipGetLastError());
    return 0;
}

int x3d_xscan_transeq_np(x3d_backend *b, real_t *rhs, const real_t *u, const real_t *conv, real_t nu,
                         const x3d_tdsops *t1, const x3d_tdsops *t2, const x3d_tdsops *t3, int acc, int np, long pitch,
                         int dirtag, bool *done)
{
    *done = false;
    if (!xscan_ok_gen(t1) || !xscan_ok_gen(t2) || !xscan_ok_gen(t3) || t1->tab.Q != t2->tab.Q || t1->tab.Q != t3->tab.Q) return 0;
    const int Q = t1->tab.Q;
    const size_t lds = sizeof(real_t) * (3 * LT_N(Q) * 64 + 3 * CS_N(Q));
    if (lds > 160 * 1024) return 0;
    int blocks = (np + 7) / 8;
    blocks = blocks > 256 ? 256 : blocks;
    const bool same = u == conv;
    ProfScope ps(b, X3D_K_TRANSEQ_FWD, dirtag, dirtag >= 0);
    int rc;
    const bool fast = t1->tab.bulk_only && t2->tab.bulk_only && t3->tab.bulk_only && t1->n_tds == 64 * Q && Q != 6;
    const bool narrow = stencil_narrow(t1) && stencil_narrow(t2) && stencil_narrow(t3);
#define GO2(Q_, F_)                                                                                            \
    (same ? (acc ? launch_transeq<Q_, true, true, F_>(b, rhs, u, conv, nu, t1, t2, t3, np, blocks, lds, pitch)       \
                 : launch_transeq<Q_, true, false, F_>(b, rhs, u, conv, nu, t1, t2, t3, np, blocks, lds, pitch))     \
          : (acc ? launch_transeq<Q_, false, true, F_>(b, rhs, u, conv, nu, t1, t2, t3, np, blocks, lds, pitch)      \
                 : launch_transeq<Q_, false, false, F_>(b, rhs, u, conv, nu, t1, t2, t3, np, blocks, lds, pitch)))
#define GO(Q_) (fast ? (narrow ? GO2(Q_, 2) : GO2(Q_, 1)) : GO2(Q_, 0))
    if (!b->sw.xscan_p1 && fast && np % 2 == 0) {
        const int blocks2 = x3d_persistent_blocks(b, (np / 2 + 7) / 8);
#define LP2(Q_, S_, A_, N_)                                                                                    \
        do {                                                                                                   \
            X3D_LDS_OPTIN(b, (k_xscan_transeq2<Q_, S_, A_, N_>));                                              \
            hipLaunchKernelGGL((k_xscan_transeq2<Q_, S_, A_, N_>), dim3(blocks2), dim3(512), lds, b->stream, rhs, u, \
                               conv, xop_of(t1), xop_of(t2), xop_of(t3), np, pitch, nu);                       \
        } while (0)
#define LP2N(Q_, S_, A_) do { if (narrow) LP2(Q_, S_, A_, true); else LP2(Q_, S_, A_, false); } while (0)
#define LP2A(Q_, S_) do { if (acc) LP2N(Q_, S_, true); else LP2N(Q_, S_, false); } while (0)
#define LP2S(Q_) do { if (same) LP2A(Q_, true); else LP2A(Q_, false); } while (0)
        if (Q == 8) LP2S(8); else LP2S(4);
#undef LP2S
#undef LP2A
// ... 322 lines not shown
    *done = true;
    return 0;
}

int x3d_ytile_transeq3_epi(x3d_backend *b, int dir, real_t *const r[3], const real_t *const f[3], real_t nu,
                           const x3d_tdsops *der1st, const x3d_tdsops *der1st_sym, const x3d_tdsops *der2nd,
                           const x3d_tdsops *der2nd_sym, const TileEpi epi[3], bool *done)
{
    *done = false;
    if (b->sw.no_tile3 || !x3d_ytile_applicable(b, dir, der1st, der1st_sym, der2nd)) return 0;
    if (der1st->tl_hash != der1st_sym->tl_hash || der2nd->tl_hash != der2nd_sym->tl_hash) return 0;
    const int Q = der1st->tab.Q;
    const int npw = ytile_npw(b, false);
    const bool circ = ytile_circ(b, der1st, der1st_sym, der2nd, der2nd_sym);
    const size_t lds = sizeof(real_t) * ((size_t)(circ ? 0 : 2 * LT_N(Q) * 64) + 16 * npw * (64 * Q + 4));
    const bool narrow = stencil_narrow(der1st) && stencil_narrow(der2nd);
    const bool uni = der1st->uniform && der1st_sym->uniform && der2nd->uniform && der2nd_sym->uniform;
    if (lds > 160 * 1024 || !narrow || !uni) return 0;
    const long pxy = (long)b->nxp * b->nyp;
    const int ntx = b->nx / (16 * npw), ntiles = ntx * (dir == X3D_DIR_Y ? b->nz : b->ny);
    const int blocks = x3d_persistent_blocks(b, ntiles);
    const long rstride = dir == X3D_DIR_Y ? (long)b->nxp : pxy, ostride = dir == X3D_DIR_Y ? pxy : (long)b->nxp;
    if (128 * rstride * X3D_RB >= (1L << 32)) return 0;
    static_assert(3 * sizeof(TileEpi) <= 512, "epi_dev slot");
    X3D_HIP(hipMemcpyAsync(b->epi_dev, epi, 3 * sizeof(TileEpi), hipMemcpyHostToDevice, b->stream));
    const TileHalo th{nullptr, nullptr, 0, 0, 0, 0, 0};
    {
        ProfScope ps(b, X3D_K_TRANSEQ_FWD, 0);
#define GOE(Q_, W_, C_)                                                                                         \
    do {                                                                                                        \
        X3D_LDS_OPTIN(b, (k_ytile_transeq3<Q_, true, true, false, true, true, true, W_, C_>));                  \
        hipLaunchKernelGGL((k_ytile_transeq3<Q_, true, true, false, true, true, true, W_, C_>), dim3(blocks), dim3(1024), lds, b->stream, \
                           r[0], r[1], r[2], f[0], f[1], f[2], xop_of(der1st), xop_of(der2nd), ntx, 0, ntiles, rstride, \
                           ostride, nu, th, (const TileEpi *)b->epi_dev, der1st->circ, der2nd->circ);           \
    } while (0)
#define GOEC(Q_, W_) do { if (circ) GOE(Q_, W_, true); else GOE(Q_, W_, false); } while (0)
        if (Q == 8) { if (npw == 2) GOEC(8, NPW2); else GOEC(8, 1); }
        else { if (npw == 2) GOEC(4, NPW2); else GOEC(4, 1); }
#undef GOEC
#undef GOE
    }
    X3D_HIP(hipGetLastError());
    b->n_tq3++;
    if (b->prof) {
        for (int k = 0; k < 2; k++) { ProfScope ps(b, X3D_K_TRANSEQ_FWD, 0); }
    }
    *done = true;
    return 0;
}

int x3d_xscan_transeq3(x3d_backend *b, real_t *const r[3], const real_t *const f[3], real_t nu,
                       const x3d_tdsops *der1st, const x3d_tdsops *der1st_sym, const x3d_tdsops *der2nd,
                       const x3d_tdsops *der2nd_sym, int acc, const real_t *const *upd_g, const x3d_tdsops *op_s,
                       const x3d_tdsops *op_i, real_t scale, real_t omega, const real_t *ushift, bool *done)
{
    *done = false;
    if ((omega != 0.0 || ushift) && (acc || upd_g)) return 0;
    if (!b->sw.x_tq3 || !x3d_xscan_fast_ok(der1st, der1st_sym, der2nd) || !x3d_xscan_fast_ok(der1st_sym, der1st, der2nd_sym)) return 0;
    if (der1st->tl_hash != der1st_sym->tl_hash || der2nd->tl_hash != der2nd_sym->tl_hash) return 0;
    const int Q = der1st->tab.Q, np = b->ny * b->nz;
    if (b->nx != 64 * Q || np % 2) return 0;
    const bool upd = upd_g != nullptr;
    if (upd) {
        auto ok = [&](const x3d_tdsops *t) {
            return xscan_ok(t) && t->tab.Q == Q && t->tab.bulk_only && t->n_tds == 64 * Q && t->tab.n_rhs == t->n_tds;
        };
        if (!ok(op_s) || !ok(op_i)) return 0;
    }
    const bool narrow = stencil_narrow(der1st) && stencil_narrow(der2nd) && (!upd || (stencil_narrow(op_s) && stencil_narrow(op_i)));
    const bool circ = b->sw.x_circ && narrow && der1st->circ_ok && der1st_sym->circ_ok && der2nd->circ_ok && der2nd_sym->circ_ok &&
                      (!upd || (op_s->circ_ok && op_i->circ_ok));
    const size_t lds = circ ? 0 : sizeof(real_t) * 64 * (upd ? 3 * LT_NC(Q) + LT_N(Q) : 2 * LT_N(Q));
    if (lds > 160 * 1024) return 0;
    const int blocks = x3d_persistent_blocks(b, (np / 2 + 7) / 8);
    XUpd xu{};
    if (upd) { xu.g[0] = upd_g[0]; xu.g[1] = upd_g[1]; xu.g[2] = upd_g[2]; xu.scale = scale; }
    xu.omega = omega; xu.ushift = ushift;
    const x3d_tdsops *ts = upd ? op_s : der1st, *ti = upd ? op_i : der1st;
    const Circ4 c4{{der1st->circ, der2nd->circ, ts->circ, ti->circ}};
#define GOX(Q_, A_, N_, U_, C_, X_)                                                                             \
    do {                                                                                                        \
        X3D_LDS_OPTIN(b, (k_xscan_transeq2x3<Q_, A_, N_, U_, C_, X_>));                                         \
        hipLaunchKernelGGL((k_xscan_transeq2x3<Q_, A_, N_, U_, C_, X_>), dim3(blocks), dim3(512), lds, b->stream, r[0], r[1], \
                           r[2], (real_t *)f[0], (real_t *)f[1], (real_t *)f[2], xop_of(der1st), xop_of(der2nd), np,  \
                           (long)b->nxp, nu, xu, xop_of(ts), xop_of(ti), c4);                                   \
    } while (0)
#define GO(Q_, A_, N_, U_, C_) do { if ((N_) && circ) GOX(Q_, A_, true, U_, C_, true); else GOX(Q_, A_, N_, U_, C_, false); } while (0)
#define GOU(Q_, A_, N_) do { if (upd) GO(Q_, A_, N_, true, false); else GO(Q_, A_, N_, false, false); } while (0)
#define GON(Q_, A_) do { if (narrow) GOU(Q_, A_, true); else GOU(Q_, A_, false); } while (0)
#define GOA(Q_)                                                                                                 \
    do {                                                                                                        \
        if (omega != 0.0 || ushift) { if (narrow) GO(Q_, false, true, false, true); else GO(Q_, false, false, false, true); } \
        else if (acc) GON(Q_, true);                                                                            \
        else GON(Q_, false);                                                                                    \
    } while (0)
    {
        ProfScope ps(b, X3D_K_TRANSEQ_FWD, X3D_DIR_X);
        if (Q == 8) GOA(8); else GOA(4);
    }
#undef GOA
#undef GON
#undef GOU
#undef GO
#undef GOX
    X3D_HIP(hipGetLastError());
    b->n_tq3++;
    if (upd) b->n_upd++;
    if (b->prof) {
        for (int k = 0; k < 2; k++) { ProfScope ps(b, X3D_K_TRANSEQ_FWD, X3D_DIR_X); }
    }
    *done = true;
    return 0;
}

int x3d_xscan_tds_lincomb(x3d_backend *b, real_t *du, const x3d_tdsops *t, real_t *y, const real_t *base, int nterm,
                          const real_t *c, const real_t *const *x, const real_t *wall, bool *done)
{
    *done = false;
    if (b->sw.no_tds_lincomb || !b->sw.x_fast || !xscan_ok(t)) return 0;
    const int Q = t->tab.Q;
    if (!(t->tab.bulk_only && t->n_tds == 64 * Q && t->tab.n_rhs == t->n_tds && b->nx == 64 * Q)) return 0;
    const int np = b->ny * b->nz;
    const bool narrow = stencil_narrow(t);
    const bool circ = narrow && t->uniform && t->circ_ok && !b->sw.no_circ;
    const size_t lds = circ ? 0 : sizeof(real_t) * LT_N(Q) * 64;
    int blocks = (np + 7) / 8;
    const int cap = circ ? 1024 : 768;
    blocks = blocks > cap ? cap : blocks;
    LinRows lr;
    lr.y = y; lr.base = base; lr.n = nterm; lr.wall = wall; lr.ny = b->ny;
    for (int k = 0; k < 5; k++) { lr.x[k] = k < nterm ? x[k] : x[0]; lr.c[k] = k < nterm ? c[k] : 0.0; }
    ProfScope ps(b, X3D_K_TDS_FWD, X3D_DIR_X);
#define GO(Q_, N_, C_) hipLaunchKernelGGL((k_xscan_tds_lin<Q_, N_, C_>), dim3(blocks), dim3(512), lds, b->stream, du, lr, xop_of(t), np, (long)b->nxp, t->circ)
    if (Q == 8) { if (circ) GO(8, true, true); else if (narrow) GO(8, true, false); else GO(8, false, false); }
    else { if (circ) GO(4, true, true); else if (narrow) GO(4, true, false); else GO(4, false, false); }
#undef GO
    X3D_HIP(hipGetLastError());
    *done = true;
    return 0;
}
```

### x3d2_amd/csrc/zfirst.hip

```cpp
#include <vector>

#include "fft_util.h"
#include "poisson_priv.h"
#include "zfft_tile.h"

#define ZH_PX 520

int x3d_ztile_fft_run(x3d_backend *b, real_t *f, const ZfArg &zf, bool fwd, int y0, int nyr);

__global__ void __launch_bounds__(256)
    k_zh_rw(real_t *__restrict__ rwZ, const real_t *__restrict__ waves, int nx, int ny, int nxs, int packed)
{
    __shared__ real_t t[32][33];
    const int kz = blockIdx.z, x0 = blockIdx.x * 32, y0 = blockIdx.y * 32;
    const int tx = threadIdx.x & 31, ty = threadIdx.x >> 5;
    for (int r = ty; r < 32; r += 8) {
        const int x = x0 + tx, y = y0 + r;
        const int xm = packed ? (x < 2 ? x * (nx / 2) : x >> 1) : (x <= nx / 2 ? x : nx - x);
        const real_t wv = waves[((size_t)kz * ny + y) * nxs + xm];
        t[r][tx] = wv < 1.e-16 ? 0.0 : -1.0 / wv;
    }
    __syncthreads();
    for (int r = ty; r < 32; r += 8) rwZ[((size_t)kz * nx + x0 + r) * ny + y0 + tx] = t[tx][r];
}
// ... 255 lines not shown
            ProfScope ps(b, X3D_K_FFT, 1);
            hipLaunchKernelGGL((k_c2c1024_x<-1>), dim3(blocks), dim3(512), lds, b->stream, p->c, x3d_fft512_twiddles(), g_tw1024,
                               nrows, (long)ZH010_PX);
        }
        bool done = false;
        {
            ProfScope ps(b, X3D_K_SPECTRAL);
            if (int rc = x3d_y010_run(b, p->c, ZH010_PX, p->nx, p->ny, p->nz, 3, p->ab, p->sym, p->luz, &done, 257)) return rc;
            X3D_REQUIRE(done, "x3d_poisson_zfirst_middle: y pass refused");
        }
        {
            ProfScope ps(b, X3D_K_SPECTRAL);
            if (int rc = x3d_y010_run(b, p->c, ZH010_PX, p->nx, p->ny, p->nz, 4, p->ab, p->sym, p->luz, &done, 257)) return rc;
            X3D_REQUIRE(done, "x3d_poisson_zfirst_middle: y pass refused");
        }
        ProfScope ps(b, X3D_K_FFT, 2);
        hipLaunchKernelGGL((k_c2c1024_x<1>), dim3(blocks), dim3(512), lds, b->stream, p->c, x3d_fft512_twiddles(), g_tw1024,
                           nrows, (long)ZH010_PX);
        X3D_HIP(hipGetLastError());
        return 0;
    }
    const real_t *rw;
    if (int rc = zh_table(p, false, &rw)) return rc;
    if (int rc = c2c_x<-1>(p, 0, 257)) return rc;
    if (int rc = x3d_fft512_run_zh(p->b, p->c, ZH_PX, 0, 257, rw, p->ab, p->nx, p->ny, p->nz)) return rc;
    return c2c_x<1>(p, 0, 257);
}

extern "C" int x3d_poisson_xfft_ok(x3d_poisson *p, int *ok)
{
    X3D_RANGE(__func__);
    X3D_REQUIRE(p && ok, "x3d_poisson_xfft_ok: null argument");
    *ok = 0;
    if (p->ext_middle || p->stretched || p->b->sw.no_xfft_div) return 0;
    bool o = false;
    if (int rc = x3d_zfirst_arg(p, nullptr, &o)) return rc;
    *ok = o ? 1 : 0;
    return 0;
}
extern "C" int x3d_poisson_zfirst_middle_xpacked(x3d_poisson *p)
{
    X3D_RANGE(__func__);
    X3D_REQUIRE(p, "x3d_poisson_zfirst_middle_xpacked: null argument");
    int ok = 0;
    if (int rc = x3d_poisson_xfft_ok(p, &ok)) return rc;
    X3D_REQUIRE(ok, "x3d_poisson_zfirst_middle_xpacked: not on offer for this solver (x3d_poisson_xfft_ok)");
    X3D_LAZY_EAGER(p->b);
    const real_t *rw;
    if (int rc = zh_table(p, true, &rw)) return rc;
    if (int rc = x3d_fft512_run_zh(p->b, p->c, ZH_PX, 0, 257, rw, p->ab, p->nx, p->ny, p->nz)) return rc;
    return c2c_x<1, true>(p, 0, 257);
}

extern "C" int x3d_poisson_create_proxy(x3d_backend *b, x3d_poisson **out, x3d_real *spectrum, int ny, long px,
                                        int (*middle)(void *), void *user)
{
    X3D_RANGE(__func__);
    X3D_REQUIRE(b && out && spectrum && middle && ny > 0 && px >= b->nx, "x3d_poisson_create_proxy: bad argument");
    X3D_REQUIRE(b->nz == 512 && b->nx % 16 == 0 && ny <= b->ny, "x3d_poisson_create_proxy: 512-row z pencils");
    x3d_poisson *p = new x3d_poisson();
    memset(p, 0, sizeof *p);
    p->b = b;
    p->nx = b->nx; p->ny = ny; p->nz = 512;
    p->ext_middle = middle; p->ext_user = user;
    p->ext_c = reinterpret_cast<real2_t *>(spectrum); p->ext_ny = ny; p->ext_px = px;
    if (int rc = x3d_fft512_init()) return rc;
    *out = p;
    return 0;
}
int x3d_proxy_hook(x3d_poisson *p, int which, real_t *f)
{
    if (which == 1) return p->ext_middle(p->ext_user);
    ZfArg zf{p->ext_c, x3d_fft512_twiddles(), p->ext_ny, p->ext_px, 0};
    return x3d_ztile_fft_run(p->b, f, zf, which == 0, 0, -1);
}

int x3d_ztile_fft_run(x3d_backend *b, real_t *f, const ZfArg &zf, bool fwd, int y0, int nyr)
{
    X3D_REQUIRE(b->nz == 512 && b->nx % 16 == 0 && zf.ny <= b->ny && zf.permn == 0, "x3d_ztile_fft_run: 512-row z pencils");
    if (nyr < 0) { y0 = 0; nyr = zf.ny; }
    X3D_REQUIRE(y0 >= 0 && y0 + nyr <= zf.ny, "x3d_ztile_fft_run: rows [%d, %d) of %d", y0, y0 + nyr, zf.ny);
    if (nyr == 0) return 0;
    const int ntx = b->nx / 16, ntiles = ntx * nyr, tile0 = ntx * y0;
    const size_t lds = sizeof(real_t) * (ZF_AREA_DOUBLES + 512);
    const long pxy = (long)b->nxp * b->nyp;
    ProfScope ps(b, X3D_K_FFT, 3);
    if (fwd) {
        X3D_LDS_OPTIN(b, (k_ztile_fft<true>));
        hipLaunchKernelGGL((k_ztile_fft<true>), dim3(ntiles < 512 ? ntiles : 512), dim3(1024), lds, b->stream, f, zf, ntx, tile0, ntiles, pxy, (long)b->nxp);
    } else {
        X3D_LDS_OPTIN(b, (k_ztile_fft<false>));
        hipLaunchKernelGGL((k_ztile_fft<false>), dim3(ntiles < 512 ? ntiles : 512), dim3(1024), lds, b->stream, f, zf, ntx, tile0, ntiles, pxy, (long)b->nxp);
    }
    X3D_HIP(hipGetLastError());
    return 0;
}

static int ztile(x3d_poisson *p, real_t *f, bool fwd)
{
    ZfArg zf;
    bool ok = false;
    if (int rc = x3d_zfirst_arg(p, &zf, &ok)) return rc;
    X3D_REQUIRE(ok && !p->stretched, "x3d_poisson_zfirst: not a 512^3 all-periodic solver (x3d_poisson_zfirst_ok)");
    return x3d_ztile_fft_run(p->b, f, zf, fwd, 0, -1);
}

// ... 38 lines not shown
```

### x3d2_amd/poisson_fft.py

```python
import ctypes
import math

import numpy as np

from . import _lib
from .common import CELL, X3dError

VP = ctypes.c_void_p


def wave_numbers(n, L, d, periodic, c_a, c_b, c_alpha):
    pi = 4.0 * math.atan(1.0)
    i = np.arange(1, n + 1, dtype=np.float64)
    if periodic:
        a, b = np.sin((i - 1) * pi / n), np.cos((i - 1) * pi / n)
    else:
        a, b = np.sin((i - 1) * pi / 2 / n), np.cos((i - 1) * pi / 2 / n)
    k, e, k2 = np.zeros(n), np.zeros(n), np.zeros(n)

    def mod_wave(w):
        wp = c_a * 2 * d * np.sin(0.5 * w) + c_b * 2 * d * np.sin(1.5 * w)
        return wp / (1.0 + 2 * c_alpha * np.cos(w))

    if periodic:
# ... 274 lines not shown
    def fft_forward(self, f_in):
        _lib.check(self.backend.lib.x3d_poisson_fft_forward(self.h, f_in.ptr))

    def fft_postprocess_000(self):
        _lib.check(self.backend.lib.x3d_poisson_postprocess_000(self.h))

    def fft_backward(self, f_out):
        _lib.check(self.backend.lib.x3d_poisson_fft_backward(self.h, f_out.ptr))

    def poisson_000(self, f, temp):
        if type(self) is HipPoissonFFT and not getattr(self.backend, "lazy", False):
            _lib.check(self.backend.lib.x3d_poisson_solve_000(self.h, f.ptr))
            return
        self.fft_forward(f)
        self.fft_postprocess_000()
        self.fft_backward(f)

    def fft_postprocess_010(self):
        _lib.check(self.backend.lib.x3d_poisson_postprocess_010(self.h))

    def enforce_periodicity_y(self, f_out, f_in):
        _lib.check(self.backend.lib.x3d_poisson_enforce_periodicity_y(self.h, f_out.ptr, f_in.ptr))

    def undo_periodicity_y(self, f_out, f_in):
        _lib.check(self.backend.lib.x3d_poisson_undo_periodicity_y(self.h, f_out.ptr, f_in.ptr))

    def poisson_010(self, f, temp):
        if temp is None:
            raise X3dError("poisson_010 needs a scratch block")
        self.enforce_periodicity_y(temp, f)
        self.solve_interleaved(temp)
        self.undo_periodicity_y(f, temp)

    def solve_poisson(self, f, temp):
        self.poisson(f, temp)

    def zfirst_ok(self):
        if type(self) is not HipPoissonFFT or self.case not in ("000", "010") or getattr(self.backend, "lazy", False):
            return False
        ok = ctypes.c_int(0)
        _lib.check(self.backend.lib.x3d_poisson_zfirst_ok(self.h, ctypes.byref(ok)))
        return bool(ok.value)

    def zfirst_middle(self):
        _lib.check(self.backend.lib.x3d_poisson_zfirst_middle(self.h))

    def xfft_ok(self):
        if not self.zfirst_ok() or self.case != "000":
            return False
        ok = ctypes.c_int(0)
        _lib.check(self.backend.lib.x3d_poisson_xfft_ok(self.h, ctypes.byref(ok)))
        return bool(ok.value)

    def zfirst_middle_xpacked(self):
        _lib.check(self.backend.lib.x3d_poisson_zfirst_middle_xpacked(self.h))

    def zfirst_forward(self, f):
        _lib.check(self.backend.lib.x3d_poisson_zfirst_forward(self.h, f.ptr))

    def zfirst_backward(self, f):
        _lib.check(self.backend.lib.x3d_poisson_zfirst_backward(self.h, f.ptr))

    def solve_zfirst(self, f):
        _lib.check(self.backend.lib.x3d_poisson_solve_000_zfirst(self.h, f.ptr))

    def interleaved_rows(self):
        if type(self) is HipPoissonFFT and self.case == "010" and self.ny_glob % 2 == 0:
            return self.ny_glob
        return 0

    def solve_interleaved(self, f):
        if getattr(self.backend, "lazy", False):
            self.fft_forward(f)
            self.fft_postprocess_010()
            self.fft_backward(f)
            return
        _lib.check(self.backend.lib.x3d_poisson_solve_010_rows(self.h, f.ptr))

    def solve_interleaved_zfirst(self, f):
        _lib.check(self.backend.lib.x3d_poisson_solve_010_rows_zfirst(self.h, f.ptr))

    def get_spectral(self):
        out = np.empty((self.nz_spec, self.ny_spec, self.nx_spec), dtype=np.complex64 if _lib.SINGLE else np.complex128)
        _lib.check(self.backend.lib.x3d_poisson_get_spectral(
            self.h, out.view(_lib.NP_REAL).ctypes.data_as(_lib.c_double_p)))
        return out

    def set_spectral(self, c):
        c = np.ascontiguousarray(c, dtype=np.complex64 if _lib.SINGLE else np.complex128)
        _lib.check(self.backend.lib.x3d_poisson_set_spectral(
            self.h, c.view(_lib.NP_REAL).ctypes.data_as(_lib.c_double_p)))


class HipPoissonFFT100(HipPoissonFFT):

    def _create(self):
        backend, mesh = self.backend, self.mesh
        lib = backend.lib
        if mesh.nproc > 1:
            raise X3dError("Multiple ranks are not yet supported for non-periodic BCs!")
        nx, ny, nz = self.nx_glob, self.ny_glob, self.nz_glob
        tb = VP()
        vd = [int(v) for v in mesh.vert_dims]
        _lib.check(lib.x3d_backend_create(ctypes.byref(tb), _lib.ints(vd[1], vd[0], vd[2]), backend.device.index,
                                          VP(backend.stream.cuda_stream)))
        self.tb = tb
        self.t1, self.t2 = VP(), VP()
        _lib.check(lib.x3d_block_alloc(tb, ctypes.byref(self.t1)))
# ... 640 lines not shown
```

### x3d2_amd/solver.py

```python
import numpy as np

from .common import (BC_DIRICHLET, BC_NEUMANN, CELL, DIR_C, DIR_X, DIR_Y, DIR_Z, RDR_C2Z, RDR_X2Y, RDR_X2Z,
                     RDR_Y2Z, RDR_Z2C, RDR_Z2X, VERT, Y_FACE, X3dError)
from .tdsops import Dirps
from .time_integrator import TimeIntegrator
from .vector_calculus import VectorCalculus


class SolverConfig:

    def __init__(self, Re=1600.0, dt=1e-3, n_iters=10, n_output=0, time_intg="RK3", poisson_solver_type="FFT",
                 der1st_scheme="compact6", der2nd_scheme="compact6", interpl_scheme="classic",
                 stagder_scheme="compact6", lowmem_transeq=False, fused=False, n_species=0, pr_species=None,
                 ibm_on=False):
        self.Re, self.dt, self.n_iters, self.n_output = Re, dt, n_iters, n_output
        self.time_intg, self.poisson_solver_type = time_intg, poisson_solver_type
        self.der1st_scheme, self.der2nd_scheme = der1st_scheme, der2nd_scheme
        self.interpl_scheme, self.stagder_scheme = interpl_scheme, stagder_scheme
        self.lowmem_transeq = lowmem_transeq
        self.n_species = int(n_species)
        self.pr_species = [1.0] * self.n_species if pr_species is None else [float(x) for x in pr_species]
        self.fused = fused
        self.ibm_on = bool(ibm_on)

# ... 32 lines not shown
        self.xdirps, self.ydirps, self.zdirps = Dirps(DIR_X), Dirps(DIR_Y), Dirps(DIR_Z)
        self.vector_calculus = VectorCalculus(backend)
        al = backend.allocator
        self.u, self.v, self.w = (al.get_block(DIR_X) for _ in range(3))
        self.nvars = 3
        self.nspecies = int(getattr(cfg, "n_species", 0))
        self.species = []
        self.nu_species = []
        if self.nspecies > 0:
            if len(cfg.pr_species) != self.nspecies:
                raise X3dError("pr_species needs one entry per species")
            self.nvars += self.nspecies
            self.nu_species = [1.0 / cfg.Re / pr for pr in cfg.pr_species]
            self.species = [al.get_block(DIR_X) for _ in range(self.nspecies)]
        self.fused = bool(cfg.fused)
        if self.fused and getattr(backend, "lazy", False):
            raise X3dError("deferred execution (HipBackend(lazy=True)) is for the op-granular driver: the fused driver "
                           "already issues the fused kernels itself and swaps block buffers behind the library's back")
        self.time_integrator = TimeIntegrator(backend, al, cfg.time_intg, self.nvars, fused=self.fused)
        self.dt, self.nu = cfg.dt, 1.0 / cfg.Re
        self.n_iters, self.n_output = cfg.n_iters, cfg.n_output
        self.ngrid = int(np.prod(mesh.get_global_dims(VERT)))
        self.current_iter = 0
        for dp in (self.xdirps, self.ydirps, self.zdirps):
            allocate_tdsops(dp, backend, mesh, cfg.der1st_scheme, cfg.der2nd_scheme, cfg.interpl_scheme,
                            cfg.stagder_scheme)
        if cfg.poisson_solver_type == "FFT":
            backend.init_poisson_fft(mesh, self.xdirps, self.ydirps, self.zdirps)
            self.poisson = self.poisson_fft
        elif cfg.poisson_solver_type == "CG":
            self.poisson = self.poisson_cg
        else:
            raise X3dError('poisson_solver_type is not valid. Use "FFT" or "CG".')
        self.pending_grad = None
        ns = self.time_integrator.nstage
        e = self.sw.epi3_stages
        self._epi3_stages = {int(v) for v in e.split(",")} if e else set(range(1, ns + 1))
        self.n_epi3 = 0
        self.rot_request, self.rot_applied = 0.0, False
        self.n_rot_fused = self.n_interleaved = 0
        self.n_zfirst = 0
        pf = backend.poisson_fft if cfg.poisson_solver_type == "FFT" else None
        self._zfirst = bool(pf is not None and getattr(pf, "zfirst_ok", lambda: False)())
        if self._zfirst:
            z = self.zdirps
            self._zfirst = (backend.zfirst_pairs_ok(z.interpl_v2p, z.stagder_v2p)
                            and backend.zfirst_pairs_ok(z.interpl_p2v, z.stagder_p2v))
        x = self.xdirps
        self._xfft_div = bool(self._zfirst and getattr(pf, "xfft_ok", lambda: False)()
                              and not hasattr(pf, "zfirst_solve_pipelined") and backend.comm.size == 1
                              and not any(backend._decomposed(d) for d in (DIR_X, DIR_Y, DIR_Z))
                              and backend.tds_apply_xfft_ok(x.stagder_v2p) and backend.tds_apply_xfft_ok(x.interpl_v2p))
        self.n_xfft_div = 0
        self.shift_request = None
        self.pending_walls = None
        self.mean_request, self._mean_ready, self.n_mean_taken = None, None, 0
        backend.before_read.append(self.flush_grad)
        self.lowmem_transeq = bool(getattr(cfg, "lowmem_transeq", False))
        if self.fused:
            self.transeq = self.transeq_fused
        else:
            self.transeq = self.transeq_lowmem if self.lowmem_transeq else self.transeq_default
        if self.fused:
            self.pressure_correction = self.pressure_correction_fused
        self.ibm = None
        self.les = None
        self.keep_pressure, self.pressure, self.pressure_wanted = False, None, False

    def transeq_default(self, rhs, variables):
        b, al = self.backend, self.backend.allocator
        du, dv, dw = rhs[:3]
        u, v, w = variables[:3]
        b.transeq_x(du, dv, dw, u, v, w, self.nu, self.xdirps)
        u_y, v_y, w_y, du_y, dv_y, dw_y = (al.get_block(DIR_Y) for _ in range(6))
        b.reorder(u_y, u, RDR_X2Y)
        b.reorder(v_y, v, RDR_X2Y)
        b.reorder(w_y, w, RDR_X2Y)
        b.transeq_y(du_y, dv_y, dw_y, u_y, v_y, w_y, self.nu, self.ydirps)
        for f in (u_y, v_y, w_y):
            al.release_block(f)
        b.sum_yintox(du, du_y)
        b.sum_yintox(dv, dv_y)
        b.sum_yintox(dw, dw_y)
        for f in (du_y, dv_y, dw_y):
            al.release_block(f)
        u_z, v_z, w_z, du_z, dv_z, dw_z = (al.get_block(DIR_Z) for _ in range(6))
        b.reorder(u_z, u, RDR_X2Z)
        b.reorder(v_z, v, RDR_X2Z)
        b.reorder(w_z, w, RDR_X2Z)
        b.transeq_z(du_z, dv_z, dw_z, u_z, v_z, w_z, self.nu, self.zdirps)
        for f in (u_z, v_z, w_z):
            al.release_block(f)
        b.sum_zintox(du, du_z)
        b.sum_zintox(dv, dv_z)
        b.sum_zintox(dw, dw_z)
        for f in (du_z, dv_z, dw_z):
            al.release_block(f)
        if self.nspecies > 0:
            self.transeq_species(rhs[3:], variables)

    def transeq_lowmem(self, rhs, variables):
        b, al = self.backend, self.backend.allocator
        du, dv, dw = rhs[:3]
        u, v, w = variables[:3]
        b.transeq_x(du, dv, dw, u, v, w, self.nu, self.xdirps)
        u_y, v_y, w_y = (al.get_block(DIR_Y) for _ in range(3))
# ... 20 lines not shown
        b.sum_zintox(du, du_z)
        b.sum_zintox(dv, dv_z)
        b.sum_zintox(dw, dw_z)
        for f in (du_z, dv_z, dw_z):
            al.release_block(f)
        u, v, w = (al.get_block(DIR_X) for _ in range(3))
        b.reorder(u, u_z, RDR_Z2X)
        b.reorder(v, v_z, RDR_Z2X)
        b.reorder(w, w_z, RDR_Z2X)
        for f in (u_z, v_z, w_z):
            al.release_block(f)
        variables[0], variables[1], variables[2] = u, v, w
        self.u, self.v, self.w = u, v, w
        if self.nspecies > 0:
            self.transeq_species(rhs[3:], variables)

    def transeq_species(self, rhs, variables):
        b, al = self.backend, self.backend.allocator
        u, v, w = variables[:3]
        for i, r in enumerate(rhs):
            b.transeq_species(r, u, variables[3 + i], self.nu_species[i], self.xdirps, i <= 0)
        for vel, dirps, rdr, summ in ((v, self.ydirps, RDR_X2Y, b.sum_yintox), (w, self.zdirps, RDR_X2Z, b.sum_zintox)):
            d = dirps.dir
            vel_d, spec_d, dspec_d = (al.get_block(d) for _ in range(3))
            b.reorder(vel_d, vel, rdr)
            for i, r in enumerate(rhs):
                b.reorder(spec_d, variables[3 + i], rdr)
                b.transeq_species(dspec_d, vel_d, spec_d, self.nu_species[i], dirps, i <= 0)
                summ(r, dspec_d)
            for f in (vel_d, spec_d, dspec_d):
                al.release_block(f)

    def transeq_species_fused(self, rhs, variables):
        b = self.backend
        vel = variables[:3]
        for i, r in enumerate(rhs):
            spec = variables[3 + i]
            for k, dirps in enumerate((self.xdirps, self.ydirps, self.zdirps)):
                b.transeq_species(r, vel[k], spec, self.nu_species[i], dirps, i <= 0, accumulate=k > 0,
                                  direction=dirps.dir)
            r.set_data_loc(spec.data_loc)

    def transeq_fused(self, rhs, variables, defer=False):
        b = self.backend
        du, dv, dw = rhs[:3]
        u, v, w = variables[:3]
        b.mesh.get_n(DIR_X, u.data_loc)
        rot, self.rot_request, self.rot_applied = self.rot_request, 0.0, False
        shift, self.shift_request = self.shift_request, None
        x = self.xdirps
        served = False
        if self.pending_grad is not None:
            g, self.pending_grad = self.pending_grad, None
            if rot != 0.0 or shift is not None:
                if not self.sw.no_rot_fused and \
                        b.transeq_x_update_rot(du, dv, dw, u, v, w, self.nu, x, g, x.stagder_p2v, x.interpl_p2v, -1.0, rot, shift):
                    served = True
                    if rot != 0.0:
                        self.rot_applied = True
                        self.n_rot_fused += 1
            elif b.transeq_x_update(du, dv, dw, u, v, w, self.nu, x, g, x.stagder_p2v, x.interpl_p2v, -1.0):
                served = True
            if not served:
                self._apply_grad(g, u, v, w)
            for f in g:
                b.allocator.release_block(f)
        if served:
            pass
        elif (rot != 0.0 or shift is not None) and not self.sw.no_rot_fused and \
                b.transeq_x_rot(du, dv, dw, u, v, w, self.nu, self.xdirps, rot, shift):
            if rot != 0.0:
                self.rot_applied = True
                self.n_rot_fused += 1
        else:
            if shift is not None:
                b.field_shift_by(u, shift)
            b.transeq_dir(DIR_X, du, dv, dw, u, v, w, self.nu, self.xdirps, accumulate=False)
        if b._decomposed(DIR_Y) or b._decomposed(DIR_Z):
            self._transeq_yz_decomposed(du, dv, dw, u, v, w)
            for f in rhs[:3]:
                f.set_data_loc(u.data_loc)
            if self.nspecies > 0:
                self.transeq_species_fused(rhs[3:], variables)
            return None
        b.transeq_dir(DIR_Y, du, dv, dw, u, v, w, self.nu, self.ydirps, accumulate=True)
        pending = None
        ti = self.time_integrator
        defer = defer and not (rot != 0.0 and not self.rot_applied)
        if (defer and not self.sw.no_defer and not self.sw.no_epi3
                and not b._decomposed(DIR_Z) and self.nspecies == 0
                and ti.istage in self._epi3_stages and b.transeq_stage_ok(DIR_Z, self.zdirps)):
            pending = {"tile3": (DIR_Z, self.nu, self.zdirps)}
            for f in rhs[:3]:
                f.set_data_loc(u.data_loc)
            return pending
        if defer and not self.sw.no_defer and not b._decomposed(DIR_Z):
            if b.transeq_stage_ok(DIR_Z, self.zdirps):
                if not self.sw.stage_in_tile:
                    pending = None
                else:
                    pending = {du.data.data_ptr(): ("tile", DIR_Z, 1, u.ptr, w.ptr, self.nu, self.zdirps),
                               dv.data.data_ptr(): ("tile", DIR_Z, 1, v.ptr, w.ptr, self.nu, self.zdirps),
                               dw.data.data_ptr(): ("tile", DIR_Z, 0, w.ptr, w.ptr, self.nu, self.zdirps)}
            else:
                al = b.allocator
                pend = [al.get_block(DIR_X) for _ in range(3)]
                if b.transeq_dir_defer(DIR_Z, pend, u, v, w, self.nu, self.zdirps):
                    pending = {r.data.data_ptr(): ("copies", pf, DIR_Z) for r, pf in zip((du, dv, dw), pend)}
                else:
                    for pf in pend:
                        al.release_block(pf)
        if pending is None:
            b.transeq_dir(DIR_Z, du, dv, dw, u, v, w, self.nu, self.zdirps, accumulate=True)
        for f in rhs[:3]:
            f.set_data_loc(u.data_loc)
        if self.nspecies > 0:
            self.transeq_species_fused(rhs[3:], variables)
# ... 30 lines not shown
        upd = self.time_integrator.pending_update
        walls, self.pending_walls = self.pending_walls or (None, None, None), None
        mean, self.mean_request, self._mean_ready = self.mean_request, None, None
        want_p = self.keep_pressure and self.pressure_wanted
        xfft = self._xfft_div and not want_p and mean is None and all(wl is None for wl in walls)
        for out, fld, op, wall in ((t1, u, x.stagder_v2p, walls[0]), (t2, v, x.interpl_v2p, walls[1]),
                                   (t3, w, x.interpl_v2p, walls[2])):
            if xfft:
                spec = upd.pop(fld.data.data_ptr(), None)
                if spec is not None:
                    b.lincomb(*spec)
                b.tds_apply_xfft(out, fld if spec is None else spec[0], op)
                continue
            spec = upd.pop(fld.data.data_ptr(), None)
            take_mean = fld is u and mean is not None and defer_grad and b.comm.size == 1 and not b._decomposed(DIR_X)
            if spec is None:
                if wall is not None:
                    b.field_set_face_from_field(fld, wall, 0.0, Y_FACE)
                if take_mean:
                    sh = b.tds_apply_mean(out, fld, op, DIR_X, mean)
                    self._mean_ready = (u.data.data_ptr(), float(mean), sh, b.red_epoch)
                else:
                    b.tds_apply(out, fld, op, DIR_X)
            elif take_mean:
                sh = b.tds_lincomb(out, op, DIR_X, *spec, wall=wall, mean_target=mean)
                self._mean_ready = (u.data.data_ptr(), float(mean), sh, b.red_epoch)
            else:
                b.tds_lincomb(out, op, DIR_X, *spec, wall=wall)
        self.time_integrator.flush_updates()
        div = t1
        jy = [(0, a1, None, t1, t2, y.interpl_v2p, y.stagder_v2p),
              (2, a2, None, t3, None, y.interpl_v2p, None)]
        jz = [(0, div, None, a1, a2, z.interpl_v2p, z.stagder_v2p)]
        nil = 0
        if self.cfg.poisson_solver_type == "FFT" and not b._decomposed(DIR_Y):
            nil = getattr(b.poisson_fft, "interleaved_rows", lambda: 0)()
        if self._zfirst and not want_p and b._decomposed(DIR_Y) and not b._decomposed(DIR_Z):
            b.tds_jobs(DIR_Y, jy)
            if self._zfirst_solve(a1, a2, t2, t3):
                b.tds_jobs(DIR_Y, [(1, a1, a2, t2, None, y.interpl_p2v, y.stagder_p2v),
                                   (2, t1, None, t3, None, y.interpl_p2v, None)])
                return self._finish_pressure_correction(u, v, w, (t1, t2, t3, a1, a2), defer_grad)
            b.tds_jobs(DIR_Z, jz)
        elif b._decomposed(DIR_Y) or b._decomposed(DIR_Z):
            nil = nil if nil and not want_p and self._zpairs_interleave(nil, jz[0]) else 0
            if nil:
                jz = [(0, t2, None, a1, a2, z.interpl_v2p, z.stagder_v2p)]
                div = t2
                self.n_interleaved += 1
            self._div_grad_decomposed(jy, jz, forward=True, nil=nil)
        else:
            b.tds_pair(*jy[0], DIR_Y)
            b.tds_apply(a2, t3, y.interpl_v2p, DIR_Y)
            if self._zfirst and not want_p and self._zfirst_solve(a1, a2, t2, t3, xpacked=xfft):
                b.tds_pair(1, a1, a2, t2, None, y.interpl_p2v, y.stagder_p2v, DIR_Y)
                b.tds_apply(t1, t3, y.interpl_p2v, DIR_Y)
                return self._finish_pressure_correction(u, v, w, (t1, t2, t3, a1, a2), defer_grad)
            if nil and not want_p and b.tds_pair_yperm(0, t2, None, a1, a2, z.interpl_v2p, z.stagder_v2p, nil):
                div = t2
                self.n_interleaved += 1
            else:
                nil = 0
                b.tds_pair(*jz[0], DIR_Z)
        p = div
        if nil:
            b.poisson_fft.solve_interleaved(p)
        elif self.cfg.poisson_solver_type == "FFT":
            b.poisson_fft.solve_poisson(p, t2)
        else:
            p.fill(0.0)
        if want_p:
            if self.pressure is None:
                self.pressure = al.get_block(DIR_X, CELL)
            b.veccopy(self.pressure, p)
        if nil and b._decomposed(DIR_Z):
            jz = [(1, t1, t3, p, None, z.interpl_p2v, z.stagder_p2v)]
            jy = [(1, a1, a2, t1, None, y.interpl_p2v, y.stagder_p2v),
                  (2, t2, None, t3, None, y.interpl_p2v, None)]
            self._div_grad_decomposed(jy, jz, forward=False, nil=nil)
            t1, t2 = t2, t1
        elif nil:
            if not b.tds_pair_yperm(1, t1, t3, p, None, z.interpl_p2v, z.stagder_p2v, nil):
                raise X3dError("pressure_correction: the interleaving z pair served the divergence but not the gradient")
            b.tds_pair(1, a1, a2, t1, None, y.interpl_p2v, y.stagder_p2v, DIR_Y)
            b.tds_apply(t2, t3, y.interpl_p2v, DIR_Y)
            t1, t2 = t2, t1
        else:
            jz = [(1, t2, t3, p, None, z.interpl_p2v, z.stagder_p2v)]
            jy = [(1, a1, a2, t2, None, y.interpl_p2v, y.stagder_p2v),
                  (2, t1, None, t3, None, y.interpl_p2v, None)]
            if b._decomposed(DIR_Y) or b._decomposed(DIR_Z):
                self._div_grad_decomposed(jy, jz, forward=False)
            else:
                b.tds_pair(*jz[0], DIR_Z)
                b.tds_pair(*jy[0], DIR_Y)
                b.tds_apply(t1, t3, y.interpl_p2v, DIR_Y)
        self._finish_pressure_correction(u, v, w, (t1, t2, t3, a1, a2), defer_grad)

    def _zfirst_solve(self, a1, a2, t2, t3, xpacked=False):
        b, z = self.backend, self.zdirps
        if xpacked:
            if not b.tds_pair_zfirst(0, None, None, a1, a2, z.interpl_v2p, z.stagder_v2p):
                raise X3dError("pressure_correction: x-transformed operands, but the z-first pair declined the divergence")
            b.poisson_fft.zfirst_middle_xpacked()
            if not b.tds_pair_zfirst(1, t2, t3, None, None, z.interpl_p2v, z.stagder_p2v):
                raise X3dError("pressure_correction: the z-first pair served the divergence but not the gradient")
            self.n_zfirst += 1
            self.n_xfft_div += 1
            return True
        pipe = getattr(b.poisson_fft, "zfirst_solve_pipelined", None)
        if pipe is not None and not b._decomposed(DIR_Z) and \
                pipe(a1, a2, t2, t3, z.interpl_v2p, z.stagder_v2p, z.interpl_p2v, z.stagder_p2v):
            self.n_zfirst += 1
            return True
        if not b.tds_pair_zfirst(0, None, None, a1, a2, z.interpl_v2p, z.stagder_v2p):
            return False
        b.poisson_fft.zfirst_middle()
        if not b.tds_pair_zfirst(1, t2, t3, None, None, z.interpl_p2v, z.stagder_p2v):
            raise X3dError("pressure_correction: the z-first pair served the divergence but not the gradient")
        self.n_zfirst += 1
        return True

    def _finish_pressure_correction(self, u, v, w, blocks, defer_grad):
        al = self.backend.allocator
        t1, t2, t3, a1, a2 = blocks
        if (defer_grad and not self.sw.no_defer and not self.sw.no_defer_grad
                and self.nspecies == 0):
            self.pending_grad = (a1, a2, t1)
            for f in (t2, t3):
                al.release_block(f)
            return
        self._apply_grad((a1, a2, t1), u, v, w)
        for f in (t1, t2, t3, a1, a2):
            al.release_block(f)

    def _zpairs_interleave(self, nil, jz0):
        b, z = self.backend, self.zdirps
        if b._decomposed(DIR_Y) or not b._decomposed(DIR_Z) or int(b.mesh.vert_dims[2]) <= 2 * 4:
            return False
        back = (1, jz0[1], jz0[4], jz0[3], None, z.interpl_p2v, z.stagder_p2v)
        return b.tds_tile_ok(DIR_Z, jz0, True, yperm=nil) and b.tds_tile_ok(DIR_Z, back, True, yperm=nil)

    def _div_grad_decomposed(self, jy, jz, forward, nil=0):
        b = self.backend
        ly, lz = not b._decomposed(DIR_Y), not b._decomposed(DIR_Z)
        nz = int(b.mesh.vert_dims[2])
        if forward:
            if ly and not lz and nz > 2 * 4 and b.tds_tile_ok(DIR_Z, jz[0], True):
                state = {}
                b.tds_jobs(DIR_Y, jy, lead=[(0, 4), (nz - 4, 4)],
                           after_lead=lambda: state.update(h=[b.tds_halo_begin(DIR_Z, j, k) for k, j in enumerate(jz)]))
                hb = [b.tds_halo_main(DIR_Z, j, k, state["h"][k], yperm=nil) for k, j in enumerate(jz)]
                for k, j in enumerate(jz):
                    b.tds_halo_finish(DIR_Z, j, k, hb[k], yperm=nil)
            else:
                if nil:
                    raise X3dError("divergence: the interleaving z pair was promised (_zpairs_interleave) but not taken")
                b.tds_jobs(DIR_Y, jy)
                b.tds_jobs(DIR_Z, jz)
            return
        if ly and not lz and b.tds_tile_ok(DIR_Z, jz[0], True) and all(b.tds_tile_ok(DIR_Y, j, False) for j in jy):
            ws, we = b.halo_strip_rows(jz[0][5], jz[0][6])
            if ws + we < nz:
                def interior():
                    for j in jy:
                        b.tds_tile_planes(DIR_Y, j, ws, nz - ws - we)
                b.tds_jobs(DIR_Z, jz, between=interior, yperm=nil)
                for j in jy:
                    b.tds_tile_planes(DIR_Y, j, 0, ws)
                    b.tds_tile_planes(DIR_Y, j, nz - we, we)
                return
        b.tds_jobs(DIR_Z, jz, yperm=nil)
        b.tds_jobs(DIR_Y, jy)

    def _apply_grad(self, g, u, v, w):
        b, x = self.backend, self.xdirps
        b.tds_apply(u, g[0], x.stagder_p2v, DIR_X, accumulate=True, scale=-1.0)
        b.tds_apply(v, g[1], x.interpl_p2v, DIR_X, accumulate=True, scale=-1.0)
        b.tds_apply(w, g[2], x.interpl_p2v, DIR_X, accumulate=True, scale=-1.0)

    def take_mean_shift(self, f, target):
        r, self._mean_ready = self._mean_ready, None
        if (r is None or self.pending_grad is None or r[0] != f.data.data_ptr() or r[1] != float(target)
                or r[3] != self.backend.red_epoch):
            return None
        self.n_mean_taken += 1
        return r[2]

    def flush_grad(self):
        if self.pending_grad is not None:
            g, self.pending_grad = self.pending_grad, None
            self._apply_grad(g, self.u, self.v, self.w)
            for f in g:
                self.backend.allocator.release_block(f)

    def divergence_v2p(self, div_u, u, v, w):
        x, y, z = self.xdirps, self.ydirps, self.zdirps
        self.vector_calculus.divergence_v2c(div_u, u, v, w, x.stagder_v2p, x.interpl_v2p, y.stagder_v2p,
                                            y.interpl_v2p, z.stagder_v2p, z.interpl_v2p)

    def gradient_p2v(self, dpdx, dpdy, dpdz, pressure):
        x, y, z = self.xdirps, self.ydirps, self.zdirps
        self.vector_calculus.gradient_c2v(dpdx, dpdy, dpdz, pressure, x.stagder_p2v, x.interpl_p2v,
                                          y.stagder_p2v, y.interpl_p2v, z.stagder_p2v, z.interpl_p2v)

    def curl(self, o_i_hat, o_j_hat, o_k_hat, u, v, w):
        self.vector_calculus.curl(o_i_hat, o_j_hat, o_k_hat, u, v, w, self.xdirps.der1st,
                                  self.ydirps.der1st, self.zdirps.der1st)

    def velocity_gradients(self):
        b = self.backend
        grads = []
        for f in (self.u, self.v, self.w):
            for dirps, d in ((self.xdirps, DIR_X), (self.ydirps, DIR_Y), (self.zdirps, DIR_Z)):
                g = b.allocator.get_block(DIR_X, VERT)
                b.tds_apply(g, f, dirps.der1st, d)
                grads.append(g)
        return grads

    def pressure_vert(self, t1, t2):
        b = self.backend
        if self.pressure is None:
            raise X3dError("compute_pressure_vert: pressure not yet computed")
        b.tds_apply(t1, self.pressure, self.zdirps.interpl_p2v, DIR_Z)
        b.tds_apply(t2, t1, self.ydirps.interpl_p2v, DIR_Y)
        b.tds_apply(t1, t2, self.xdirps.interpl_p2v, DIR_X)
        return t1

    def poisson_fft(self, pressure, div_u):
        b, al = self.backend, self.backend.allocator
        p_temp = al.get_block(DIR_C)
        b.reorder(p_temp, div_u, RDR_Z2C)
        temp = al.get_block(DIR_C)
        b.poisson_fft.solve_poisson(p_temp, temp)
        al.release_block(temp)
        b.reorder(pressure, p_temp, RDR_C2Z)
        al.release_block(p_temp)

    def poisson_cg(self, pressure, div_u):
        pressure.fill(0.0)

    def pressure_correction(self, u, v, w):
        b, al = self.backend, self.backend.allocator
        div_u = al.get_block(DIR_Z)
        self.divergence_v2p(div_u, u, v, w)
# ... 18 lines not shown
```

Measured before the change: 3.552 billion DoF*steps/s.

## Keep pressure gradient in x-packed spectral form and fuse inverse x-FFT into transeq update

The Poisson middle stage can now leave the gradient operands in x-packed half-spectrum form, skipping its inverse x FFT. That inverse 512-point real FFT is folded into the x-direction gradient application, both in a standalone kernel and inside the fused transeq-x update kernel, where it is applied to the packed rows before the circulant solve. This removes a separate full-field inverse FFT pass and its memory round trip. In exchange, the wavefront-level FFT work and twiddle LDS usage move into the register-heavy transeq kernel, which could reduce its occupancy.

```diff
diff --git a/include/x3d2_hip.h b/include/x3d2_hip.h
--- a/include/x3d2_hip.h
+++ b/include/x3d2_hip.h
@@ -274,6 +274,15 @@
 int x3d_poisson_xfft_ok(x3d_poisson *p, int *ok);
 int x3d_poisson_zfirst_middle_xpacked(x3d_poisson *p);
 int x3d_c2c512_x_rows(x3d_backend *b, x3d_real *c, long nrows, long pitch, int mode);
+int x3d_tds_solve_ixfft_ok(x3d_backend *b, const x3d_tdsops *t, int *ok);
+int x3d_tds_solve_ixfft(x3d_backend *b, x3d_real *u, const x3d_real *g, const x3d_tdsops *t, x3d_real scale);
+int x3d_transeq_x_update_xinv_ok(x3d_backend *b, const x3d_tdsops *op_u, const x3d_tdsops *op_vw, int *ok);
+int x3d_transeq_x_update_xinv(x3d_backend *b, x3d_real *du, x3d_real *dv, x3d_real *dw, x3d_real *u, x3d_real *v, x3d_real *w,
+                              x3d_real nu, const x3d_tdsops *der1st, const x3d_tdsops *der1st_sym, const x3d_tdsops *der2nd,
+                              const x3d_tdsops *der2nd_sym, const x3d_real *gu, const x3d_real *gv, const x3d_real *gw,
+                              const x3d_tdsops *op_u, const x3d_tdsops *op_vw, x3d_real scale, int *done);
+int x3d_poisson_xfft_grad_ok(x3d_poisson *p, int *ok);
+int x3d_poisson_zfirst_middle_xpacked2(x3d_poisson *p);
 int x3d_poisson_set_stretching_zfirst(x3d_poisson *p, int sym, const x3d_real *a0, const x3d_real *a1);
 int x3d_poisson_create_proxy(x3d_backend *b, x3d_poisson **out, x3d_real *spectrum, int ny, long px, int (*middle)(void *user),
                              void *user);
diff --git a/x3d2_amd/_lib.py b/x3d2_amd/_lib.py
--- a/x3d2_amd/_lib.py
+++ b/x3d2_amd/_lib.py
@@ -184,6 +184,12 @@
     "x3d_poisson_xfft_ok": (I, [VP, c_int_p]),
     "x3d_poisson_zfirst_middle_xpacked": (I, [VP]),
     "x3d_c2c512_x_rows": (I, [VP, VP, ctypes.c_long, ctypes.c_long, I]),
+    "x3d_tds_solve_ixfft_ok": (I, [VP, VP, c_int_p]),
+    "x3d_tds_solve_ixfft": (I, [VP, VP, VP, VP, D]),
+    "x3d_transeq_x_update_xinv_ok": (I, [VP, VP, VP, c_int_p]),
+    "x3d_transeq_x_update_xinv": (I, [VP, VP, VP, VP, VP, VP, VP, D, VP, VP, VP, VP, VP, VP, VP, VP, VP, D, c_int_p]),
+    "x3d_poisson_xfft_grad_ok": (I, [VP, c_int_p]),
+    "x3d_poisson_zfirst_middle_xpacked2": (I, [VP]),
     "x3d_tds_pair_zfirst": (I, [VP, VP, I, VP, VP, VP, VP, VP, VP, c_int_p]),
     "x3d_sfftz_create": (I, [VP, ctypes.POINTER(VP), c_int_p, I, I, I]),
     "x3d_sfftz_destroy": (I, [VP]),
diff --git a/x3d2_amd/backend.py b/x3d2_amd/backend.py
--- a/x3d2_amd/backend.py
+++ b/x3d2_amd/backend.py
@@ -491,6 +491,23 @@
                                                  op_u.handle, op_vw.handle, float(scale), ctypes.byref(flag)))
         return bool(flag.value)
 
+    def transeq_x_update_xinv_ok(self, op_u, op_vw):
+        if self._decomposed(DIR_X):
+            return False
+        flag = ctypes.c_int(0)
+        _lib.check(self.lib.x3d_transeq_x_update_xinv_ok(self.h, op_u.handle, op_vw.handle, ctypes.byref(flag)))
+        return bool(flag.value)
+
+    def transeq_x_update_xinv(self, du, dv, dw, u, v, w, nu, dirps, grads, op_u, op_vw, scale):
+        if self._decomposed(DIR_X):
+            return False
+        flag = ctypes.c_int(0)
+        _lib.check(self.lib.x3d_transeq_x_update_xinv(self.h, du.ptr, dv.ptr, dw.ptr, u.ptr, v.ptr, w.ptr, float(nu),
+                                                      dirps.der1st.handle, dirps.der1st_sym.handle, dirps.der2nd.handle,
+                                                      dirps.der2nd_sym.handle, grads[0].ptr, grads[1].ptr, grads[2].ptr,
+                                                      op_u.handle, op_vw.handle, float(scale), ctypes.byref(flag)))
+        return bool(flag.value)
+
     def transeq_x_update_rot(self, du, dv, dw, u, v, w, nu, dirps, grads, op_u, op_vw, scale, omega, u_shift=None):
         if self._decomposed(DIR_X):
             return False
@@ -662,6 +679,16 @@
 
     def tds_apply_xfft(self, du, u, tdsops):
         _lib.check(self.lib.x3d_tds_solve_xfft(self.h, du.ptr, u.ptr, tdsops.handle))
+
+    def tds_apply_ixfft_ok(self, tdsops):
+        if self._decomposed(DIR_X):
+            return False
+        flag = ctypes.c_int(0)
+        _lib.check(self.lib.x3d_tds_solve_ixfft_ok(self.h, tdsops.handle, ctypes.byref(flag)))
+        return bool(flag.value)
+
+    def tds_apply_ixfft(self, du, g, tdsops, scale):
+        _lib.check(self.lib.x3d_tds_solve_ixfft(self.h, du.ptr, g.ptr, tdsops.handle, float(scale)))
 
     def tds_apply(self, du, u, tdsops, direction, accumulate=False, scale=1.0):
         if not self._decomposed(direction):
diff --git a/x3d2_amd/csrc/common.h b/x3d2_amd/csrc/common.h
--- a/x3d2_amd/csrc/common.h
+++ b/x3d2_amd/csrc/common.h
@@ -108,7 +108,7 @@
 struct x3d_switches {
     long no_via_x, no_xscan, no_ygen, no_ytile, no_q5, no_direct, sfft010_split_xy;
     long no_circ, no_halo_circ, no_uniform, xscan_p1, no_ztile, no_tds_pair, no_npw2, no_tile3, xdir_generic, no_xcirc;
-    long no_tds_lincomb, no_zfirst010, no_zfirst, no_xwide, no_xwide_upd, no_xfft_div;
+    long no_tds_lincomb, no_zfirst010, no_zfirst, no_xwide, no_xwide_upd, no_xfft_div, no_xfft_grad;
     long no_spectral_pad, no_fft512, no_rwt, no_r2c512, no_y010, y010_no_db, no_onchip2, no_slab_fused_z;
     long lazy_dump, lazy_report, lazy_keep_zero_terms;
     long pad_x;
diff --git a/x3d2_amd/csrc/fft512_core.h b/x3d2_amd/csrc/fft512_core.h
--- a/x3d2_amd/csrc/fft512_core.h
+++ b/x3d2_amd/csrc/fft512_core.h
@@ -142,3 +142,40 @@
     }
     wave_lds_fence();
 }
+
+__device__ __forceinline__ void load_packed(real2_t (&g)[4], const real_t *__restrict__ row, int l)
+{
+    const real2_t *__restrict__ g2 = reinterpret_cast<const real2_t *>(row);
+#pragma unroll
+    for (int f = 0; f < 4; f++) g[f] = g2[l + 64 * f];
+}
+__device__ __forceinline__ void irfft512_packed_wave(const real2_t (&g)[4], real_t (&r)[8], real2_t *__restrict__ pen,
+                                                     const real2_t *__restrict__ tw, int l)
+{
+    real2_t a[4];
+    wave_lds_fence();
+#pragma unroll
+    for (int f = 0; f < 4; f++) pen[l + 64 * f] = g[f];
+    wave_lds_fence();
+#pragma unroll
+    for (int f = 0; f < 4; f++) {
+        const int k = l + 64 * f;
+        const real2_t c = pen[(256 - k) & 255];
+        const real2_t wk = twiddle<1>(tw, k);
+        const real_t sx = g[f].x + c.x, sy = g[f].y - c.y;
+        const real_t dx = g[f].x - c.x, dy = g[f].y + c.y;
+        a[f] = make_real2(sx - fma_r(wk.x, dy, wk.y * dx), sy + fma_r(wk.x, dx, -(wk.y * dy)));
+        if (f == 0) a[f] = l == 0 ? make_real2(g[0].x + g[0].y, g[0].x - g[0].y) : a[f];
+    }
+    fft256_wave<1>(a, pen, tw, l);
+    const int wsw = (l >> 2) & 3, rsw = (l >> 4) & 3;
+#pragma unroll
+    for (int f = 0; f < 4; f++) pen[64 * f + ((l & ~3) | ((l & 3) ^ rsw))] = a[f];
+    wave_lds_fence();
+#pragma unroll
+    for (int q = 0; q < 4; q++) {
+        const real2_t v = pen[4 * l + (q ^ wsw)];
+        r[2 * q] = v.x;
+        r[2 * q + 1] = v.y;
+    }
+}
diff --git a/x3d2_amd/csrc/switches.hip b/x3d2_amd/csrc/switches.hip
--- a/x3d2_amd/csrc/switches.hip
+++ b/x3d2_amd/csrc/switches.hip
@@ -42,6 +42,7 @@
     F("X3D_NO_R2C512", no_r2c512),
     F("X3D_NO_ZFIRST", no_zfirst),
     F("X3D_NO_XFFT_DIV", no_xfft_div),
+    F("X3D_NO_XFFT_GRAD", no_xfft_grad),
     F("X3D_NO_ZFIRST010", no_zfirst010),
     F("X3D_NO_Y010", no_y010),
     F("X3D_Y010_NO_DB", y010_no_db),
diff --git a/x3d2_amd/csrc/tds.hip b/x3d2_amd/csrc/tds.hip
--- a/x3d2_amd/csrc/tds.hip
+++ b/x3d2_amd/csrc/tds.hip
@@ -798,7 +798,8 @@
 int x3d_xscan_transeq3(x3d_backend *b, real_t *const r[3], const real_t *const f[3], real_t nu,
                        const x3d_tdsops *der1st, const x3d_tdsops *der1st_sym, const x3d_tdsops *der2nd,
                        const x3d_tdsops *der2nd_sym, int acc, const real_t *const *upd_g, const x3d_tdsops *op_s,
-                       const x3d_tdsops *op_i, real_t scale, real_t omega, const real_t *ushift, bool *done);
+                       const x3d_tdsops *op_i, real_t scale, real_t omega, const real_t *ushift, bool *done,
+                       bool xinv = false);
 int x3d_xwide_transeq3_upd(x3d_backend *b, real_t *const r[3], real_t *const f[3], real_t nu, const x3d_tdsops *der1st,
                            const x3d_tdsops *der1st_sym, const x3d_tdsops *der2nd, const x3d_tdsops *der2nd_sym,
                            const real_t *const g[3], const x3d_tdsops *op_s, const x3d_tdsops *op_i, real_t scale,
@@ -935,6 +936,26 @@
     X3D_REQUIRE(du != u, "x3d_tds_solve_xfft: du and u must be distinct blocks");
     if (int rc = check_len(b, t, X3D_DIR_X, "tds_solve_xfft")) return rc;
     return x3d_xscan_tds_xfft(b, du, u, t);
+}
+
+bool x3d_xscan_tds_ixfft_ok(const x3d_backend *b, const x3d_tdsops *t);
+int x3d_xscan_tds_ixfft(x3d_backend *b, real_t *du, const real_t *g, const x3d_tdsops *t, real_t scale);
+extern "C" int x3d_tds_solve_ixfft_ok(x3d_backend *b, const x3d_tdsops *t, int *ok)
+{
+    X3D_RANGE(__func__);
+    X3D_REQUIRE(b && t && ok, "x3d_tds_solve_ixfft_ok: null argument");
+    *ok = x3d_xscan_tds_ixfft_ok(b, t) ? 1 : 0;
+    return 0;
+}
+extern "C" int x3d_tds_solve_ixfft(x3d_backend *b, real_t *du, const real_t *g, const x3d_tdsops *t, real_t scale)
+{
+    X3D_RANGE(__func__);
+    if (b) X3D_LAZY_SYNC(b);
+    X3D_LAZY_EAGER(b);
+    X3D_REQUIRE(b && du && g && t, "x3d_tds_solve_ixfft: null argument");
+    X3D_REQUIRE(du != g, "x3d_tds_solve_ixfft: du and g must be distinct blocks");
+    if (int rc = check_len(b, t, X3D_DIR_X, "tds_solve_ixfft")) return rc;
+    return x3d_xscan_tds_ixfft(b, du, g, t, scale);
 }
 
 int x3d_ytile_tds_pair(x3d_backend *b, int dir, int mode, real_t *out1, real_t *out2, const real_t *in1, const real_t *in2,
@@ -1355,6 +1376,42 @@
     return 0;
 }
 
+extern "C" int x3d_transeq_x_update_xinv_ok(x3d_backend *b, const x3d_tdsops *op_u, const x3d_tdsops *op_vw, int *ok)
+{
+    X3D_RANGE(__func__);
+    X3D_REQUIRE(b && op_u && op_vw && ok, "x3d_transeq_x_update_xinv_ok: null argument");
+    *ok = b->sw.x_tq3 && b->sw.x_circ && x3d_xscan_tds_ixfft_ok(b, op_u) && x3d_xscan_tds_ixfft_ok(b, op_vw) ? 1 : 0;
+    return 0;
+}
+extern "C" int x3d_transeq_x_update_xinv(x3d_backend *b, real_t *du, real_t *dv, real_t *dw, real_t *u, real_t *v, real_t *w,
+                                         real_t nu, const x3d_tdsops *der1st, const x3d_tdsops *der1st_sym,
+                                         const x3d_tdsops *der2nd, const x3d_tdsops *der2nd_sym, const real_t *gu,
+                                         const real_t *gv, const real_t *gw, const x3d_tdsops *op_u,
+                                         const x3d_tdsops *op_vw, real_t scale, int *done)
+{
+    X3D_RANGE(__func__);
+    if (b) X3D_LAZY_SYNC(b);
+    X3D_LAZY_EAGER(b);
+    X3D_REQUIRE(b && du && dv && dw && u && v && w && der1st && der1st_sym && der2nd && der2nd_sym && gu && gv && gw &&
+                    op_u && op_vw && done,
+                "x3d_transeq_x_update_xinv: null argument");
+    *done = 0;
+    if (int rc = transeq_check(b, X3D_DIR_X, der1st, der1st_sym, der2nd)) return rc;
+    if (int rc = check_len(b, op_u, X3D_DIR_X, "transeq_x_update_xinv")) return rc;
+    if (int rc = check_len(b, op_vw, X3D_DIR_X, "transeq_x_update_xinv")) return rc;
+    real_t *r[3] = {du, dv, dw};
+    const real_t *f[3] = {u, v, w}, *g[3] = {gu, gv, gw};
+    for (int c = 0; c < 3; c++)
+        for (int k = 0; k < 3; k++)
+            X3D_REQUIRE(r[c] != f[k] && r[c] != g[k] && f[c] != g[k], "x3d_transeq_x_update_xinv: arguments alias");
+    bool ok = false;
+    if (int rc = x3d_xscan_transeq3(b, r, f, nu, der1st, der1st_sym, der2nd, der2nd_sym, 0, g, op_u, op_vw, scale, 0.0,
+                                    nullptr, &ok, true))
+        return rc;
+    *done = ok ? 1 : 0;
+    return 0;
+}
+
 extern "C" int x3d_transeq_x_update_rot(x3d_backend *b, real_t *du, real_t *dv, real_t *dw, real_t *u, real_t *v, real_t *w,
                                         real_t nu, const x3d_tdsops *der1st, const x3d_tdsops *der1st_sym,
                                         const x3d_tdsops *der2nd, const x3d_tdsops *der2nd_sym, const real_t *gu,
diff --git a/x3d2_amd/csrc/xscan.hip b/x3d2_amd/csrc/xscan.hip
--- a/x3d2_amd/csrc/xscan.hip
+++ b/x3d2_amd/csrc/xscan.hip
@@ -201,6 +201,32 @@
     }
 }
 
+__global__ void __launch_bounds__(512, 4) k_xscan_tds_ixfft(real_t *__restrict__ du, const real_t *__restrict__ g, int np,
+                                                            long pitch, real_t scale, CircOp co,
+                                                            const real2_t *__restrict__ twg)
+{
+    constexpr int Q = 8;
+    extern __shared__ real2_t xf[];
+    real2_t *__restrict__ tws = xf + 8 * FP256;
+    if (threadIdx.x < 256) tws[threadIdx.x] = twg[threadIdx.x];
+    __syncthreads();
+    const int lane = threadIdx.x & 63;
+    const int wave = __builtin_amdgcn_readfirstlane(threadIdx.x >> 6);
+    real2_t *__restrict__ pen = xf + wave * FP256;
+    const int nwaves = gridDim.x * (blockDim.x >> 6);
+    const int p0 = blockIdx.x * (blockDim.x >> 6) + wave;
+    real2_t ng[4];
+    if (p0 < np) load_packed(ng, g + (long)p0 * pitch, lane);
+    for (int p = p0; p < np; p += nwaves) {
+        real_t b[Q], w[Q + 8], r[Q];
+        irfft512_packed_wave(ng, b, pen, tws, lane);
+        if (p + nwaves < np) load_packed(ng, g + (long)(p + nwaves) * pitch, lane);
+        window_from_body<Q>(w, b, lane);
+        circ_solve<Q, true>(w, r, co, lane);
+        store_rows_q8<true>(du + (long)p * pitch, lane, r, scale);
+    }
+}
+
 template <int Q, bool NARROW, bool CIRC = false>
 __global__ void __launch_bounds__(512) k_xscan_tds_lin(real_t *__restrict__ du, LinRows lr, XOp t, int np, long pitch,
                                                        CircOp co)
@@ -471,15 +497,25 @@
     const real_t *ushift;
 };
 
-template <int Q, bool ACC, bool NARROW, bool UPD, bool CHN = false, bool CIRC = false>
+template <int Q, bool ACC, bool NARROW, bool UPD, bool CHN = false, bool CIRC = false, bool XINV = false>
 __global__ void __launch_bounds__(512)
     k_xscan_transeq2x3(real_t *__restrict__ rhs0, real_t *__restrict__ rhs1, real_t *__restrict__ rhs2, real_t *u0,
                        real_t *u1, real_t *u2, XOp tD1, XOp tD2, int np, long pitch, real_t nu, XUpd upd, XOp tS,
-                       XOp tI, Circ4 cc)
+                       XOp tI, Circ4 cc, const real2_t *__restrict__ twg = nullptr)
 {
     extern __shared__ real_t lt[];
     constexpr int LNF = LT_N(Q) * 64, LNC = LT_NC(Q) * 64, L1N = UPD ? LNC : LNF;
     static_assert(!CIRC || NARROW, "CIRC: 5-tap stencils");
+    static_assert(!XINV || (UPD && CIRC && Q == 8 && !CHN), "XINV: the circulant UPD form on 512-row pencils");
+    real2_t *__restrict__ xpen = nullptr;
+    const real2_t *__restrict__ tws = nullptr;
+    if constexpr (XINV) {
+        real2_t *__restrict__ xf = reinterpret_cast<real2_t *>(lt);
+        if (threadIdx.x < 256) xf[8 * FP256 + threadIdx.x] = twg[threadIdx.x];
+        __syncthreads();
+        tws = xf + 8 * FP256;
+        xpen = xf + __builtin_amdgcn_readfirstlane(threadIdx.x >> 6) * FP256;
+    }
     if constexpr (!CIRC) {
         for (int i = threadIdx.x; i < L1N; i += blockDim.x) lt[i] = tD1.TL[i];
         for (int i = threadIdx.x; i < LNF; i += blockDim.x) lt[L1N + i] = tD2.TL[i];
@@ -498,9 +534,14 @@
     const real_t *__restrict__ l1 = lt, *__restrict__ l3 = lt + L1N;
     real_t na[Q], nb[Q];
     const int pstart = 2 * (blockIdx.x * (blockDim.x >> 6) + wave);
+    real2_t ga[XINV ? 4 : 1], gb[XINV ? 4 : 1];
     if (pstart < np) {
         load_body<Q>(na, u0 + (long)pstart * pitch, lane);
         load_body<Q>(nb, u0 + (long)(pstart + 1) * pitch, lane);
+        if constexpr (XINV) {
+            load_packed(ga, upd.g[0] + (long)pstart * pitch, lane);
+            load_packed(gb, upd.g[0] + (long)(pstart + 1) * pitch, lane);
+        }
     }
     for (int p = pstart; p < np; p += 2 * nwaves) {
         V2 cb[Q];
@@ -522,13 +563,27 @@
                     }
                 }
                 if constexpr (UPD) {
-                    const real_t *gsrc = (c == 0 ? upd.g[0] : (c == 1 ? upd.g[1] : upd.g[2])) + (long)p * pitch;
-                    real_t ga[Q], gb[Q];
-                    load_body<Q>(ga, gsrc, lane);
-                    load_body<Q>(gb, gsrc + pitch, lane);
                     V2 g2[Q], wg[Q + 8], X[Q], du1, xn;
-#pragma unroll
-                    for (int q = 0; q < Q; q++) g2[q] = V2{ga[q], gb[q]};
+                    if constexpr (XINV) {
+                        real_t ra_[Q], rb_[Q];
+                        irfft512_packed_wave(ga, ra_, xpen, tws, lane);
+                        irfft512_packed_wave(gb, rb_, xpen, tws, lane);
+#pragma unroll
+                        for (int q = 0; q < Q; q++) g2[q] = V2{ra_[q], rb_[q]};
+                        const real_t *gn = c == 0 ? upd.g[1] + (long)p * pitch : (c == 1 ? upd.g[2] + (long)p * pitch
+                                                                                    : upd.g[0] + (long)(pn < np ? pn : p) * pitch);
+                        if (c < 2 || pn < np) {
+                            load_packed(ga, gn, lane);
+                            load_packed(gb, gn + pitch, lane);
+                        }
+                    } else {
+                        const real_t *gsrc = (c == 0 ? upd.g[0] : (c == 1 ? upd.g[1] : upd.g[2])) + (long)p * pitch;
+                        real_t ga_[Q], gb_[Q];
+                        load_body<Q>(ga_, gsrc, lane);
+                        load_body<Q>(gb_, gsrc + pitch, lane);
+#pragma unroll
+                        for (int q = 0; q < Q; q++) g2[q] = V2{ga_[q], gb_[q]};
+                    }
                     window_from_body<Q, V2>(wg, g2, lane);
                     if constexpr (CIRC) {
                         if (c == 0) circ_solve<Q, NARROW, V2>(wg, X, cc.o[2], lane);
@@ -1435,6 +1490,25 @@
     blocks = blocks > 1024 ? 1024 : blocks;
     ProfScope ps(b, X3D_K_TDS_FWD, X3D_DIR_X);
     hipLaunchKernelGGL(k_xscan_tds_xfft, dim3(blocks), dim3(512), lds, b->stream, du, u, np, (long)b->nxp, t->circ,
+                       x3d_fft512_twiddles());
+    X3D_HIP(hipGetLastError());
+    return 0;
+}
+
+bool x3d_xscan_tds_ixfft_ok(const x3d_backend *b, const x3d_tdsops *t)
+{
+    return x3d_xscan_tds_xfft_ok(b, t) && !b->sw.no_xfft_grad;
+}
+int x3d_xscan_tds_ixfft(x3d_backend *b, real_t *du, const real_t *g, const x3d_tdsops *t, real_t scale)
+{
+    X3D_REQUIRE(x3d_xscan_tds_ixfft_ok(b, t), "x3d_tds_solve_ixfft: not on offer for this operator (x3d_tds_solve_ixfft_ok)");
+    if (int rc = x3d_fft512_init()) return rc;
+    const int np = b->ny * b->nz;
+    const size_t lds = sizeof(real2_t) * (8 * FP256 + 256);
+    int blocks = (np + 7) / 8;
+    blocks = blocks > 1024 ? 1024 : blocks;
+    ProfScope ps(b, X3D_K_TDS_FWD, X3D_DIR_X);
+    hipLaunchKernelGGL(k_xscan_tds_ixfft, dim3(blocks), dim3(512), lds, b->stream, du, g, np, (long)b->nxp, scale, t->circ,
                        x3d_fft512_twiddles());
     X3D_HIP(hipGetLastError());
     return 0;
@@ -1863,9 +1937,10 @@
 int x3d_xscan_transeq3(x3d_backend *b, real_t *const r[3], const real_t *const f[3], real_t nu,
                        const x3d_tdsops *der1st, const x3d_tdsops *der1st_sym, const x3d_tdsops *der2nd,
                        const x3d_tdsops *der2nd_sym, int acc, const real_t *const *upd_g, const x3d_tdsops *op_s,
-                       const x3d_tdsops *op_i, real_t scale, real_t omega, const real_t *ushift, bool *done)
+                       const x3d_tdsops *op_i, real_t scale, real_t omega, const real_t *ushift, bool *done, bool xinv)
 {
     *done = false;
+    if (xinv && !(upd_g && !acc && x3d_xscan_tds_ixfft_ok(b, op_s) && x3d_xscan_tds_ixfft_ok(b, op_i))) return 0;
     if ((omega != 0.0 || ushift) && (acc || upd_g)) return 0;
     if (!b->sw.x_tq3 || !x3d_xscan_fast_ok(der1st, der1st_sym, der2nd) || !x3d_xscan_fast_ok(der1st_sym, der1st, der2nd_sym)) return 0;
     if (der1st->tl_hash != der1st_sym->tl_hash || der2nd->tl_hash != der2nd_sym->tl_hash) return 0;
@@ -1881,8 +1956,13 @@
     const bool narrow = stencil_narrow(der1st) && stencil_narrow(der2nd) && (!upd || (stencil_narrow(op_s) && stencil_narrow(op_i)));
     const bool circ = b->sw.x_circ && narrow && der1st->circ_ok && der1st_sym->circ_ok && der2nd->circ_ok && der2nd_sym->circ_ok &&
                       (!upd || (op_s->circ_ok && op_i->circ_ok));
-    const size_t lds = circ ? 0 : sizeof(real_t) * 64 * (upd ? 3 * LT_NC(Q) + LT_N(Q) : 2 * LT_N(Q));
+    if (xinv && !(circ && Q == 8)) return 0;
+    const size_t lds = xinv ? sizeof(real2_t) * (8 * FP256 + 256)
+                            : (circ ? 0 : sizeof(real_t) * 64 * (upd ? 3 * LT_NC(Q) + LT_N(Q) : 2 * LT_N(Q)));
     if (lds > 160 * 1024) return 0;
+    if (xinv) {
+        if (int rc = x3d_fft512_init()) return rc;
+    }
     const int blocks = x3d_persistent_blocks(b, (np / 2 + 7) / 8);
     XUpd xu{};
     if (upd) { xu.g[0] = upd_g[0]; xu.g[1] = upd_g[1]; xu.g[2] = upd_g[2]; xu.scale = scale; }
@@ -1894,7 +1974,7 @@
         X3D_LDS_OPTIN(b, (k_xscan_transeq2x3<Q_, A_, N_, U_, C_, X_>));                                         \
         hipLaunchKernelGGL((k_xscan_transeq2x3<Q_, A_, N_, U_, C_, X_>), dim3(blocks), dim3(512), lds, b->stream, r[0], r[1], \
                            r[2], (real_t *)f[0], (real_t *)f[1], (real_t *)f[2], xop_of(der1st), xop_of(der2nd), np,  \
-                           (long)b->nxp, nu, xu, xop_of(ts), xop_of(ti), c4);                                   \
+                           (long)b->nxp, nu, xu, xop_of(ts), xop_of(ti), c4, nullptr);                          \
     } while (0)
 #define GO(Q_, A_, N_, U_, C_) do { if ((N_) && circ) GOX(Q_, A_, true, U_, C_, true); else GOX(Q_, A_, N_, U_, C_, false); } while (0)
 #define GOU(Q_, A_, N_) do { if (upd) GO(Q_, A_, N_, true, false); else GO(Q_, A_, N_, false, false); } while (0)
@@ -1907,7 +1987,12 @@
     } while (0)
     {
         ProfScope ps(b, X3D_K_TRANSEQ_FWD, X3D_DIR_X);
-        if (Q == 8) GOA(8); else GOA(4);
+        if (xinv) {
+            X3D_LDS_OPTIN(b, (k_xscan_transeq2x3<8, false, true, true, false, true, true>));
+            hipLaunchKernelGGL((k_xscan_transeq2x3<8, false, true, true, false, true, true>), dim3(blocks), dim3(512), lds,
+                               b->stream, r[0], r[1], r[2], (real_t *)f[0], (real_t *)f[1], (real_t *)f[2], xop_of(der1st),
+                               xop_of(der2nd), np, (long)b->nxp, nu, xu, xop_of(ts), xop_of(ti), c4, x3d_fft512_twiddles());
+        } else if (Q == 8) GOA(8); else GOA(4);
     }
 #undef GOA
 #undef GON
diff --git a/x3d2_amd/csrc/zfirst.hip b/x3d2_amd/csrc/zfirst.hip
--- a/x3d2_amd/csrc/zfirst.hip
+++ b/x3d2_amd/csrc/zfirst.hip
@@ -331,6 +331,27 @@
     return c2c_x<1, true>(p, 0, 257);
 }
 
+extern "C" int x3d_poisson_xfft_grad_ok(x3d_poisson *p, int *ok)
+{
+    X3D_RANGE(__func__);
+    X3D_REQUIRE(p && ok, "x3d_poisson_xfft_grad_ok: null argument");
+    if (int rc = x3d_poisson_xfft_ok(p, ok)) return rc;
+    if (p->b->sw.no_xfft_grad) *ok = 0;
+    return 0;
+}
+extern "C" int x3d_poisson_zfirst_middle_xpacked2(x3d_poisson *p)
+{
+    X3D_RANGE(__func__);
+    X3D_REQUIRE(p, "x3d_poisson_zfirst_middle_xpacked2: null argument");
+    int ok = 0;
+    if (int rc = x3d_poisson_xfft_grad_ok(p, &ok)) return rc;
+    X3D_REQUIRE(ok, "x3d_poisson_zfirst_middle_xpacked2: not on offer for this solver (x3d_poisson_xfft_grad_ok)");
+    X3D_LAZY_EAGER(p->b);
+    const real_t *rw;
+    if (int rc = zh_table(p, true, &rw)) return rc;
+    return x3d_fft512_run_zh(p->b, p->c, ZH_PX, 0, 257, rw, p->ab, p->nx, p->ny, p->nz);
+}
+
 extern "C" int x3d_poisson_create_proxy(x3d_backend *b, x3d_poisson **out, x3d_real *spectrum, int ny, long px,
                                         int (*middle)(void *), void *user)
 {
diff --git a/x3d2_amd/poisson_fft.py b/x3d2_amd/poisson_fft.py
--- a/x3d2_amd/poisson_fft.py
+++ b/x3d2_amd/poisson_fft.py
@@ -350,8 +350,18 @@
         _lib.check(self.backend.lib.x3d_poisson_xfft_ok(self.h, ctypes.byref(ok)))
         return bool(ok.value)
 
-    def zfirst_middle_xpacked(self):
-        _lib.check(self.backend.lib.x3d_poisson_zfirst_middle_xpacked(self.h))
+    def zfirst_middle_xpacked(self, out_packed=False):
+        if out_packed:
+            _lib.check(self.backend.lib.x3d_poisson_zfirst_middle_xpacked2(self.h))
+        else:
+            _lib.check(self.backend.lib.x3d_poisson_zfirst_middle_xpacked(self.h))
+
+    def xfft_grad_ok(self):
+        if not self.xfft_ok():
+            return False
+        ok = ctypes.c_int(0)
+        _lib.check(self.backend.lib.x3d_poisson_xfft_grad_ok(self.h, ctypes.byref(ok)))
+        return bool(ok.value)
 
     def zfirst_forward(self, f):
         _lib.check(self.backend.lib.x3d_poisson_zfirst_forward(self.h, f.ptr))
diff --git a/x3d2_amd/solver.py b/x3d2_amd/solver.py
--- a/x3d2_amd/solver.py
+++ b/x3d2_amd/solver.py
@@ -108,6 +108,12 @@
                               and not any(backend._decomposed(d) for d in (DIR_X, DIR_Y, DIR_Z))
                               and backend.tds_apply_xfft_ok(x.stagder_v2p) and backend.tds_apply_xfft_ok(x.interpl_v2p))
         self.n_xfft_div = 0
+        self._xfft_grad = bool(self._xfft_div and getattr(pf, "xfft_grad_ok", lambda: False)()
+                               and backend.tds_apply_ixfft_ok(x.stagder_p2v) and backend.tds_apply_ixfft_ok(x.interpl_p2v)
+                               and backend.transeq_x_update_xinv_ok(x.stagder_p2v, x.interpl_p2v))
+        self.n_xfft_grad = 0
+        self.pending_grad_packed = False
+        self._grad_packed = False
         self.shift_request = None
         self.pending_walls = None
         self.mean_request, self._mean_ready, self.n_mean_taken = None, None, 0
@@ -234,7 +240,12 @@
         served = False
         if self.pending_grad is not None:
             g, self.pending_grad = self.pending_grad, None
-            if rot != 0.0 or shift is not None:
+            packed, self.pending_grad_packed = self.pending_grad_packed, False
+            if packed:
+                if rot == 0.0 and shift is None and \
+                        b.transeq_x_update_xinv(du, dv, dw, u, v, w, self.nu, x, g, x.stagder_p2v, x.interpl_p2v, -1.0):
+                    served = True
+            elif rot != 0.0 or shift is not None:
                 if not self.sw.no_rot_fused and \
                         b.transeq_x_update_rot(du, dv, dw, u, v, w, self.nu, x, g, x.stagder_p2v, x.interpl_p2v, -1.0, rot, shift):
                     served = True
@@ -244,7 +255,7 @@
             elif b.transeq_x_update(du, dv, dw, u, v, w, self.nu, x, g, x.stagder_p2v, x.interpl_p2v, -1.0):
                 served = True
             if not served:
-                self._apply_grad(g, u, v, w)
+                self._apply_grad(g, u, v, w, packed)
             for f in g:
                 b.allocator.release_block(f)
         if served:
@@ -381,9 +392,11 @@
         else:
             b.tds_pair(*jy[0], DIR_Y)
             b.tds_apply(a2, t3, y.interpl_v2p, DIR_Y)
-            if self._zfirst and not want_p and self._zfirst_solve(a1, a2, t2, t3, xpacked=xfft):
+            xgrad = xfft and self._xfft_grad
+            if self._zfirst and not want_p and self._zfirst_solve(a1, a2, t2, t3, xpacked=xfft, xpacked_out=xgrad):
                 b.tds_pair(1, a1, a2, t2, None, y.interpl_p2v, y.stagder_p2v, DIR_Y)
                 b.tds_apply(t1, t3, y.interpl_p2v, DIR_Y)
+                self._grad_packed = xgrad
                 return self._finish_pressure_correction(u, v, w, (t1, t2, t3, a1, a2), defer_grad)
             if nil and not want_p and b.tds_pair_yperm(0, t2, None, a1, a2, z.interpl_v2p, z.stagder_v2p, nil):
                 div = t2
@@ -426,16 +439,17 @@
                 b.tds_apply(t1, t3, y.interpl_p2v, DIR_Y)
         self._finish_pressure_correction(u, v, w, (t1, t2, t3, a1, a2), defer_grad)
 
-    def _zfirst_solve(self, a1, a2, t2, t3, xpacked=False):
+    def _zfirst_solve(self, a1, a2, t2, t3, xpacked=False, xpacked_out=False):
         b, z = self.backend, self.zdirps
         if xpacked:
             if not b.tds_pair_zfirst(0, None, None, a1, a2, z.interpl_v2p, z.stagder_v2p):
                 raise X3dError("pressure_correction: x-transformed operands, but the z-first pair declined the divergence")
-            b.poisson_fft.zfirst_middle_xpacked()
+            b.poisson_fft.zfirst_middle_xpacked(out_packed=xpacked_out)
             if not b.tds_pair_zfirst(1, t2, t3, None, None, z.interpl_p2v, z.stagder_p2v):
                 raise X3dError("pressure_correction: the z-first pair served the divergence but not the gradient")
             self.n_zfirst += 1
             self.n_xfft_div += 1
+            self.n_xfft_grad += 1 if xpacked_out else 0
             return True
         pipe = getattr(b.poisson_fft, "zfirst_solve_pipelined", None)
         if pipe is not None and not b._decomposed(DIR_Z) and \
@@ -453,13 +467,15 @@
     def _finish_pressure_correction(self, u, v, w, blocks, defer_grad):
         al = self.backend.allocator
         t1, t2, t3, a1, a2 = blocks
+        packed, self._grad_packed = self._grad_packed, False
         if (defer_grad and not self.sw.no_defer and not self.sw.no_defer_grad
                 and self.nspecies == 0):
             self.pending_grad = (a1, a2, t1)
+            self.pending_grad_packed = packed
             for f in (t2, t3):
                 al.release_block(f)
             return
-        self._apply_grad((a1, a2, t1), u, v, w)
+        self._apply_grad((a1, a2, t1), u, v, w, packed)
         for f in (t1, t2, t3, a1, a2):
             al.release_block(f)
 
@@ -502,8 +518,13 @@
         b.tds_jobs(DIR_Z, jz, yperm=nil)
         b.tds_jobs(DIR_Y, jy)
 
-    def _apply_grad(self, g, u, v, w):
+    def _apply_grad(self, g, u, v, w, packed=False):
         b, x = self.backend, self.xdirps
+        if packed:
+            b.tds_apply_ixfft(u, g[0], x.stagder_p2v, -1.0)
+            b.tds_apply_ixfft(v, g[1], x.interpl_p2v, -1.0)
+            b.tds_apply_ixfft(w, g[2], x.interpl_p2v, -1.0)
+            return
         b.tds_apply(u, g[0], x.stagder_p2v, DIR_X, accumulate=True, scale=-1.0)
         b.tds_apply(v, g[1], x.interpl_p2v, DIR_X, accumulate=True, scale=-1.0)
         b.tds_apply(w, g[2], x.interpl_p2v, DIR_X, accumulate=True, scale=-1.0)
@@ -519,7 +540,8 @@
     def flush_grad(self):
         if self.pending_grad is not None:
             g, self.pending_grad = self.pending_grad, None
-            self._apply_grad(g, self.u, self.v, self.w)
+            packed, self.pending_grad_packed = self.pending_grad_packed, False
+            self._apply_grad(g, self.u, self.v, self.w, packed)
             for f in g:
                 self.backend.allocator.release_block(f)
 
```

Measured after the change: 3.629 billion DoF*steps/s, median of 6. +2.2%, better.
